# zhouxian/FluidLab

Measured on AMD Instinct MI355X. Metric: MPM substeps/sec (fwd+bwd), 128^3 grid / 200k particles, higher is better.
Workload: dtype f32; 1 GPU; water block 128^3 grid, 200k particles (BASELINE configs[1] inputs), fwd+bwd, evolving (rolling window); nc_start=34727, nc_end=99101, parallelism=1 env, 1 GPU

## Files before the change

### __graft_entry__.py

```python
import os
import subprocess
import sys

ROOT = os.path.dirname(os.path.abspath(__file__))
CSRC = os.path.join(ROOT, 'fluidlab_amd', 'csrc')
HIP_LIB = os.path.join(CSRC, 'libfluidengine_hip.so')
HIPCC_FLAGS = ['--offload-arch=gfx950', '-O3', '-std=c++17', '-shared', '-fPIC', '-munsafe-fp-atomics', '-fno-slp-vectorize']


def _hipcc():
    for c in ('/opt/rocm/bin/hipcc', 'hipcc'):
        if c == 'hipcc' or os.path.exists(c):
            return c


def _source_hash(sources):
    import hashlib
    h = hashlib.sha256(' '.join(HIPCC_FLAGS).encode())
    for s in sources:
        h.update(os.path.basename(s).encode())
        with open(s, 'rb') as f:
            h.update(f.read())
    return h.hexdigest()


def build(force=False):
    srcs = [os.path.join(CSRC, f) for f in ('fe_engine.hip', 'fe_math.h', 'fe_smoke.h', 'fe_mesh.h', 'fe_param_grad.h', 'fe_summary.h', 'fe_task_loss.h')] + \
           [os.path.join(ROOT, 'include', f) for f in ('fluidengine.h', 'fluidengine_ext.h')]
    stamp, want = HIP_LIB + '.srchash', _source_hash(srcs)
    have = open(stamp).read().strip() if os.path.exists(stamp) else ''
    if force or os.environ.get('FE_FORCE_BUILD') == '1' or not os.path.exists(HIP_LIB) or have != want:
        subprocess.check_call([_hipcc()] + HIPCC_FLAGS + ['-o', HIP_LIB, os.path.join(CSRC, 'fe_engine.hip')])
        with open(stamp, 'w') as f:
            f.write(want + '\n')
        print('build: compiled', os.path.relpath(HIP_LIB, ROOT), 'from sources', want[:16])
    else:
        print('build: up to date', os.path.relpath(HIP_LIB, ROOT), 'sources', want[:16])
    subprocess.check_call(['make', '-s', '-C', os.path.join(ROOT, 'oracle')])
    if ROOT not in sys.path:
        sys.path.insert(0, ROOT)
    import fluidlab_amd
    from fluidlab_amd import _capi
    lib = _capi.load_hip()
    missing = lib.missing_symbols()
    assert not missing, f'libfluidengine_hip.so is missing ABI symbols: {missing}'
    assert lib.has_ext, f'libfluidengine_hip.so is missing extension symbols: {lib.missing_ext_symbols()}'


def smoke():
    if ROOT not in sys.path:
        sys.path.insert(0, ROOT)
    sys.path.insert(0, os.path.join(ROOT, 'tests'))
    import numpy as np
    import scenarios as S
    from fluidlab_amd import _capi
    hip = _capi.load_hip()
    oracle = _capi.EngineLib(os.path.join(ROOT, 'oracle', '_build', 'libfe_oracle_f64.so'))
    sc = S.latte_mini()
    a = S.run_latte(hip, sc, device=0)
    b = S.run_latte(oracle, sc)
    assert (a['final']['used'] == b['final']['used']).all()
    assert S.rel_l2(a['final']['x'], b['final']['x']) <= 1e-5, S.rel_l2(a['final']['x'], b['final']['x'])
    assert S.rel_l2(a['step_loss'], b['step_loss']) <= 1e-4
    assert S.cosine(a['action_grad'], b['action_grad']) >= 0.999999
    assert S.rel_l2(a['action_grad'], b['action_grad']) <= 1e-4
    print('smoke ok: backend', hip.backend, 'loss', float(np.sum(a['step_loss'])),
          'action-grad rel L2 vs oracle', S.rel_l2(a['action_grad'], b['action_grad']))


if __name__ == '__main__':
    build(force='--force' in sys.argv)
    if len(sys.argv) > 1 and sys.argv[1] == 'smoke':
        smoke()
```

### fluidlab_amd/_capi.py

```python
import ctypes as C
import os

import numpy as np

_HERE = os.path.dirname(os.path.abspath(__file__))
HIP_LIB_PATH = os.path.join(_HERE, 'csrc', 'libfluidengine_hip.so')

FE_BOUNDARY_CUBE, FE_BOUNDARY_CYLINDER = 0, 1
FE_EFF_PLAIN, FE_EFF_INJECTOR, FE_EFF_AIRCON = 0, 1, 2


class FeEngineError(RuntimeError):
    pass


def _structs(real):
    class FeBoundary(C.Structure):
        _fields_ = [('type', C.c_int), ('lower', real * 3), ('upper', real * 3),
                    ('xz_center', real * 2), ('xz_radius', real), ('restitution', real),
                    ('lock_dims', C.c_int)]

    class FeConfig(C.Structure):
        _fields_ = [('struct_size', C.c_int), ('n_grid', C.c_int), ('n_particles', C.c_int),
                    ('max_substeps_local', C.c_int), ('n_substeps', C.c_int),
# ... 153 lines not shown
    global _hip_lib
    if _hip_lib is None:
        if not os.path.exists(HIP_LIB_PATH):
            raise FeEngineError(
                f'{HIP_LIB_PATH} is missing: build it with `python -c "import __graft_entry__ as g; g.build()"` '
                '(hipcc --offload-arch=gfx950).  There is no CPU fallback.')
        _hip_lib = EngineLib(HIP_LIB_PATH)
    return _hip_lib


class Engine:

    def __init__(self, elib, *, n_grid, n_particles, max_substeps_local, n_substeps,
                 max_action_steps, dt, p_vol, gravity, boundary, device=0):
        self.elib = elib
        self.lib = elib.lib
        self.dtype = elib.dtype
        cfg = elib.FeConfig()
        cfg.struct_size = C.sizeof(elib.FeConfig)
        cfg.n_grid = int(n_grid)
        cfg.n_particles = int(n_particles)
        cfg.max_substeps_local = int(max_substeps_local)
        cfg.n_substeps = int(n_substeps)
        cfg.max_action_steps = int(max_action_steps)
        cfg.dt = float(dt)
        cfg.p_vol = float(p_vol)
        cfg.gravity[:] = [float(g) for g in gravity]
        cfg.boundary = boundary
        cfg.device = int(device)
        self.device = int(device)
        self.cfg = cfg
        self.N = int(n_particles)
        self.n_obs = 0
        self.n_summary_groups = 0
        self.n_task_terms = 0
        self.h = self.lib.fe_create(C.byref(cfg))
        if not self.h:
            raise FeEngineError('fe_create failed: ' + self.lib.fe_last_error(None).decode())
        self.h = C.c_void_p(self.h)

    def close(self):
        if getattr(self, 'h', None):
            self.lib.fe_destroy(self.h)
            self.h = None

    def __del__(self):
        try:
            self.close()
        except Exception:
            pass

    def _ck(self, rc):
        if rc != 0:
            raise FeEngineError(self.lib.fe_last_error(self.h).decode())

    def _r(self, a, shape=None):
        if a is None:
            return None, None
        a = np.ascontiguousarray(a, dtype=self.dtype)
        if shape is not None:
            assert a.shape == tuple(shape), f'expected shape {shape}, got {a.shape}'
        return a, a.ctypes.data_as(C.c_void_p)

    def _i(self, a, shape=None):
        if a is None:
            return None, None
        a = np.ascontiguousarray(a, dtype=np.int32)
        if shape is not None:
            assert a.shape == tuple(shape), f'expected shape {shape}, got {a.shape}'
        return a, a.ctypes.data_as(C.c_void_p)

    def _out(self, a, shape, dtype=None):
        dtype = dtype or self.dtype
        assert isinstance(a, np.ndarray) and a.dtype == dtype and a.flags['C_CONTIGUOUS'] and a.shape == tuple(shape)
        return a.ctypes.data_as(C.c_void_p)

    def sync(self):
        self._ck(self.lib.fe_sync(self.h))

    def set_option(self, name, value):
        self._ck(self.lib.fe_set_option(self.h, name.encode(), float(value)))

    OPTION_NAMES = ('sort_interval', 'item_max', 'grid_store', 'p2g_grad_waves', 'g2p_grad_v', 'loose_max', 'xcd_map', 'write_through',
                    'wave_sort', 'lane_split', 'fold_reorder', 'compact_F', 'fuse_g2p', 'fuse_bwd', 'quad_min_units', 'pgg_quad_min_units', 'quad_max', 'quad_fit', 'pack_units', 'wgrid_cap', 'wgrid_cap_g2p', 'wgrid_cap_pgg', 'ggrid_cap', 'collide_type')

    def get_option(self, name):
        v = C.c_double(0.0)
        self._ck(self.lib.fe_get_option(self.h, name.encode(), C.byref(v)))
        return v.value

    def get_options(self):
        return {n: self.get_option(n) for n in self.OPTION_NAMES}

    def init_particles(self, x, used, mat, mat_cls, mu, lam, rho, body_id):
        N = self.N
        k0, x_ = self._r(x, (N, 3)); k1, u_ = self._i(used, (N,)); k2, m_ = self._i(mat, (N,))
        k3, c_ = self._i(mat_cls, (N,)); k4, mu_ = self._r(mu, (N,)); k5, la_ = self._r(lam, (N,))
        k6, rh_ = self._r(rho, (N,)); k7, b_ = self._i(body_id, (N,))
        self._ck(self.lib.fe_init_particles(self.h, x_, u_, m_, c_, mu_, la_, rh_, b_))

    def substep(self, f, f_global, act):
        self._ck(self.lib.fe_substep(self.h, int(f), int(f_global), int(bool(act))))

    def substep_grad(self, f, f_global, act):
        self._ck(self.lib.fe_substep_grad(self.h, int(f), int(f_global), int(bool(act))))

    def step(self, f0, f_global0, n, act):
        self._ck(self.lib.fe_step(self.h, int(f0), int(f_global0), int(n), int(bool(act))))

    def step_grad(self, f0, f_global0, n, act):
        self._ck(self.lib.fe_step_grad(self.h, int(f0), int(f_global0), int(n), int(bool(act))))

    def get_frame(self, f, x=None, v=None, C_=None, F=None, used=None):
        N = self.N
        px = self._out(x, (N, 3)) if x is not None else None
        pv = self._out(v, (N, 3)) if v is not None else None
        pC = self._out(C_, (N, 3, 3)) if C_ is not None else None
        pF = self._out(F, (N, 3, 3)) if F is not None else None
        pu = self._out(used, (N,), np.int32) if used is not None else None
        self._ck(self.lib.fe_get_frame(self.h, int(f), px, pv, pC, pF, pu))

    def set_frame(self, f, x=None, v=None, C_=None, F=None, used=None):
        N = self.N
        k0, px = self._r(x, (N, 3)); k1, pv = self._r(v, (N, 3)); k2, pC = self._r(C_, (N, 3, 3))
        k3, pF = self._r(F, (N, 3, 3)); k4, pu = self._i(used, (N,))
        self._ck(self.lib.fe_set_frame(self.h, int(f), px, pv, pC, pF, pu))

    @staticmethod
    def _handles(engines):
        arr = (C.c_void_p * len(engines))(*[e.h for e in engines])
        return arr

    @staticmethod
    def step_batch(engines, f0, f_global0, n, act):
        e0 = engines[0]
        e0._ck(e0.lib.fe_step_batch(Engine._handles(engines), len(engines), int(f0), int(f_global0), int(n), int(bool(act))))

    @staticmethod
    def step_grad_batch(engines, f0, f_global0, n, act):
        e0 = engines[0]
        e0._ck(e0.lib.fe_step_grad_batch(Engine._handles(engines), len(engines), int(f0), int(f_global0), int(n), int(bool(act))))

    def copy_frame(self, src, dst):
        self._ck(self.lib.fe_copy_frame(self.h, int(src), int(dst)))

    def copy_grad(self, src, dst):
        self._ck(self.lib.fe_copy_grad(self.h, int(src), int(dst)))

    def reset_grad(self):
        self._ck(self.lib.fe_reset_grad(self.h))

    def reset_grad_till_frame(self, f):
        self._ck(self.lib.fe_reset_grad_till_frame(self.h, int(f)))

    def get_grad(self, f):
        N = self.N
        gx = np.zeros((N, 3), self.dtype); gv = np.zeros((N, 3), self.dtype)
        gC = np.zeros((N, 3, 3), self.dtype); gF = np.zeros((N, 3, 3), self.dtype)
        self._ck(self.lib.fe_get_grad(self.h, int(f), gx.ctypes.data_as(C.c_void_p), gv.ctypes.data_as(C.c_void_p),
                                      gC.ctypes.data_as(C.c_void_p), gF.ctypes.data_as(C.c_void_p)))
        return gx, gv, gC, gF

    @staticmethod
    def _tptr(t):
        return None if t is None else C.c_void_p(t.data_ptr())

    def _torch_fence(self, *tensors):
# ... 243 lines not shown
        d.softness = float(softness)
        self._ck(self.lib.fe_eff_set_mesh(self.h, int(e), C.byref(d), pv))

    def eff_set_act_range(self, e, act_range):
        k, p = self._i(act_range)
        self._ck(self.lib.fe_eff_set_act_range(self.h, int(e), p, int(k.shape[0])))

    def eff_get_state(self, e, f):
        s = np.zeros((8,), self.dtype)
        self._ck(self.lib.fe_eff_get_state(self.h, int(e), int(f), s.ctypes.data_as(C.c_void_p)))
        return s

    def eff_set_state(self, e, f, state8):
        k, p = self._r(state8, (8,))
        self._ck(self.lib.fe_eff_set_state(self.h, int(e), int(f), p))

    def eff_get_vw(self, e, f):
        v = np.zeros((3,), self.dtype); w = np.zeros((3,), self.dtype)
        self._ck(self.lib.fe_eff_get_vw(self.h, int(e), int(f), v.ctypes.data_as(C.c_void_p), w.ctypes.data_as(C.c_void_p)))
        return v, w

    def eff_set_vw(self, e, f, v, w):
        k0, pv = self._r(v, (3,)); k1, pw = self._r(w, (3,))
        self._ck(self.lib.fe_eff_set_vw(self.h, int(e), int(f), pv, pw))

    def eff_set_action(self, e, s, s_global, n_substeps, action):
        k, p = self._r(action)
        self._ck(self.lib.fe_eff_set_action(self.h, int(e), int(s), int(s_global), int(n_substeps), p))

    def eff_set_action_grad(self, e, s, s_global, n_substeps):
        self._ck(self.lib.fe_eff_set_action_grad(self.h, int(e), int(s), int(s_global), int(n_substeps)))

    def eff_apply_action_p(self, e, action_p):
        k, p = self._r(action_p)
        self._ck(self.lib.fe_eff_apply_action_p(self.h, int(e), p))

    def eff_apply_action_p_grad(self, e):
        self._ck(self.lib.fe_eff_apply_action_p_grad(self.h, int(e)))

    def eff_get_action_grad(self, e, s, n, action_dim):
        g = np.zeros((n + 1, action_dim), self.dtype)
        self._ck(self.lib.fe_eff_get_action_grad(self.h, int(e), int(s), int(n), g.ctypes.data_as(C.c_void_p)))
        return g

    def agent_copy_frame(self, src, dst):
        self._ck(self.lib.fe_agent_copy_frame(self.h, int(src), int(dst)))

    def agent_copy_grad(self, src, dst):
        self._ck(self.lib.fe_agent_copy_grad(self.h, int(src), int(dst)))

    def agent_reset_grad_till_frame(self, f):
        self._ck(self.lib.fe_agent_reset_grad_till_frame(self.h, int(f)))

    def agent_set_collector(self, boundary=None, mat=-1):
        self._ck(self.lib.fe_agent_set_collector(self.h, C.byref(boundary) if boundary is not None else None, int(mat)))

    def loss_alloc(self, max_loss_steps):
        self._ck(self.lib.fe_loss_alloc(self.h, int(max_loss_steps)))

    def loss_set_target(self, s, x):
        k, p = self._r(x, (self.N, 3))
        self._ck(self.lib.fe_loss_set_target(self.h, int(s), p))

    def loss_clear(self):
        self._ck(self.lib.fe_loss_clear(self.h))

    def loss_step(self, s, f, matching_mat, weight):
        self._ck(self.lib.fe_loss_step(self.h, int(s), int(f), int(matching_mat), self.elib.real(weight)))

    def loss_step_grad(self, s, f, matching_mat, weight, step_loss_grad):
        self._ck(self.lib.fe_loss_step_grad(self.h, int(s), int(f), int(matching_mat), self.elib.real(weight),
                                            self.elib.real(step_loss_grad)))

    def loss_get(self, n):
        a = np.zeros((n,), self.dtype)
        self._ck(self.lib.fe_loss_get(self.h, a.ctypes.data_as(C.c_void_p), int(n)))
        return a

    def get_stats(self, f):
        st = FeStats()
        self._ck(self.lib.fe_get_stats(self.h, int(f), C.byref(st)))
        return {k: getattr(st, k) for k, _ in FeStats._fields_}

    def get_work_stats(self, f):
        out = (C.c_longlong * 24)()
        if hasattr(self.lib, 'fe_get_work_stats_n'):
            self._ck(self.lib.fe_get_work_stats_n(self.h, int(f), out, 24))
        else:
            self._ck(self.lib.fe_get_work_stats(self.h, int(f), out))
        keys = ('n_items', 'tail_start', 'n_active_blocks', 'n_multi_item_workgroups', 'n_single_item_blocks')
        d = {k: int(out[i]) for i, k in enumerate(keys)}
        d['items_by_size'] = {k: int(out[5 + i]) for i, k in enumerate(('1', '2-4', '5-8', '9-16', '17-32', '33-64', '65-128'))}
        d['n_occupied_blocks'] = int(out[12])
        d['n_loose_particles'] = int(out[13])
        d['n_quad_items'] = int(out[14])
        d['n_quad_units'] = int(out[15])
        d['n_scatter_units'], d['n_gather_units'] = int(out[16]), int(out[17])
        d['packed'] = bool(out[18])
        d['n_leftover_items'] = int(out[19]) + int(out[20])
        d['n_split9_waves'], d['n_split3_waves'] = int(out[21]), int(out[22])
        return d

    def timer_start(self):
        self._ck(self.lib.fe_timer_start(self.h))

    def timer_stop_ms(self):
        ms = self.lib.fe_timer_stop_ms(self.h)
        if ms < 0:
            raise FeEngineError(self.lib.fe_last_error(self.h).decode())
        return ms

    def profile_enable(self, on):
        self._ck(self.lib.fe_profile_enable(self.h, int(bool(on))))

    def profile_read(self, cap=32):
        buf = C.create_string_buffer(4096)
        ms = (C.c_double * cap)()
        cnt = (C.c_longlong * cap)()
        n = self.lib.fe_profile_read(self.h, buf, 4096, ms, cnt, cap)
        names = buf.value.decode().split('\n') if n > 0 else []
        return {names[i]: (ms[i], cnt[i]) for i in range(min(n, len(names)))}
```

### fluidlab_amd/csrc/fe_engine.hip

```cpp
#include <hip/hip_runtime.h>

#include <algorithm>
#include <cstdio>
#include <cstdlib>
#include <cstring>
#include <string>
#include <vector>

#include "../../include/fluidengine.h"
#include "../../include/fluidengine_ext.h"
#include "fe_math.h"

static_assert(sizeof(fe_real) == 4, "the HIP engine is fp32 (macros.py:207-211)");

#define FR_WORDS 25
#define GR_WORDS 24

template <typename T>
struct Plane {
    char* base; unsigned off;
    __host__ __device__ __forceinline__ T& operator[](int s) const { return *(T*)(base + (size_t)(off + (unsigned)s * (unsigned)sizeof(T))); }
    __host__ __device__ __forceinline__ T* ptr() const { return (T*)(base + (size_t)off); }
};
typedef unsigned int u32x4 __attribute__((ext_vector_type(4)));
typedef unsigned int u32x3 __attribute__((ext_vector_type(3)));
__device__ __forceinline__ __amdgpu_buffer_rsrc_t wt_rsrc(void* base) { return __builtin_amdgcn_make_buffer_rsrc(base, 0, -1, 0x00020000); }
__device__ __forceinline__ void wt_store16(void* base, unsigned byte_off, float4 v) {
    const u32x4 u = {__float_as_uint(v.x), __float_as_uint(v.y), __float_as_uint(v.z), __float_as_uint(v.w)};
    __builtin_amdgcn_raw_buffer_store_b128(u, wt_rsrc(base), (int)byte_off, 0, 16);
}
__device__ __forceinline__ void wt_store4(void* base, unsigned byte_off, unsigned v) { __builtin_amdgcn_raw_buffer_store_b32(v, wt_rsrc(base), (int)byte_off, 0, 16); }
struct FrameV {
    Plane<float4> A0, A1, A2; Plane<float> a3, a4, a5; Plane<float4> B0, B1; Plane<float> b2; Plane<int> used;
    int wt;
    int iso;
};
__device__ __forceinline__ void pstore(const FrameV& fr, const Plane<float4>& p, int s, float4 v) {
    if (fr.wt) wt_store16(p.base, p.off + (unsigned)s * 16u, v); else p[s] = v;
}
__device__ __forceinline__ void pstore(const FrameV& fr, const Plane<float>& p, int s, float v) {
    if (fr.wt) wt_store4(p.base, p.off + (unsigned)s * 4u, __float_as_uint(v)); else p[s] = v;
}
__device__ __forceinline__ void pstore(const FrameV& fr, const Plane<int>& p, int s, int v) {
    if (fr.wt) wt_store4(p.base, p.off + (unsigned)s * 4u, (unsigned)v); else p[s] = v;
}
__host__ __device__ inline FrameV frame_view(float* base_, size_t Np_, int wt = 0, int iso = 0) {
    FrameV v;
    v.wt = wt; v.iso = iso;
    char* base = (char*)base_;
    const unsigned Np = (unsigned)Np_;
    v.A0 = {base, 0u}; v.A1 = {base, 16u * Np}; v.A2 = {base, 32u * Np};
    v.a3 = {base, 48u * Np}; v.a4 = {base, 52u * Np}; v.a5 = {base, 56u * Np};
    v.B0 = {base, 60u * Np}; v.B1 = {base, 76u * Np}; v.b2 = {base, 92u * Np};
    v.used = {base, 96u * Np};
    return v;
}

struct PState { float x[3], v[3]; m3 C, F; };
__device__ __forceinline__ void copy_xvC(PState& d, const PState& s) {
#pragma unroll
    for (int a = 0; a < 3; a++) {
        d.x[a] = s.x[a]; d.v[a] = s.v[a];
#pragma unroll
        for (int b = 0; b < 3; b++) d.C.a[a][b] = s.C.a[a][b];
    }
}

__device__ __forceinline__ void load_xvC(const FrameV& fr, int s, PState& p) {
    float4 a0 = fr.A0[s], a1 = fr.A1[s], a2 = fr.A2[s];
    p.x[0] = a0.x; p.x[1] = a0.y; p.x[2] = a0.z; p.v[0] = a0.w; p.v[1] = a1.x; p.v[2] = a1.y;
    p.C.a[0][0] = a1.z; p.C.a[0][1] = a1.w; p.C.a[0][2] = a2.x; p.C.a[1][0] = a2.y; p.C.a[1][1] = a2.z; p.C.a[1][2] = a2.w;
    p.C.a[2][0] = fr.a3[s]; p.C.a[2][1] = fr.a4[s]; p.C.a[2][2] = fr.a5[s];
}
__device__ __forceinline__ void load_F(const FrameV& fr, int s, m3& F) {
    if (fr.iso) {
        const float c = fr.b2[s];
        const float d = fr.iso == 1 ? c : 0.f;
        F.a[0][0] = d; F.a[0][1] = 0.f; F.a[0][2] = 0.f; F.a[1][0] = 0.f; F.a[1][1] = d; F.a[1][2] = 0.f; F.a[2][0] = 0.f; F.a[2][1] = 0.f; F.a[2][2] = c;
        return;
    }
    float4 b0 = fr.B0[s], b1 = fr.B1[s];
    F.a[0][0] = b0.x; F.a[0][1] = b0.y; F.a[0][2] = b0.z; F.a[1][0] = b0.w;
    F.a[1][1] = b1.x; F.a[1][2] = b1.y; F.a[2][0] = b1.z; F.a[2][1] = b1.w; F.a[2][2] = fr.b2[s];
}
__device__ __forceinline__ void store_xvC(const FrameV& fr, int s, const float x[3], const float v[3], const m3& C) {
    const float4 a0 = make_float4(x[0], x[1], x[2], v[0]), a1 = make_float4(v[1], v[2], C.a[0][0], C.a[0][1]), a2 = make_float4(C.a[0][2], C.a[1][0], C.a[1][1], C.a[1][2]);
    if (fr.wt) {
        const unsigned o16 = (unsigned)s * 16u, o4 = (unsigned)s * 4u;
        wt_store16(fr.A0.base, fr.A0.off + o16, a0); wt_store16(fr.A0.base, fr.A1.off + o16, a1); wt_store16(fr.A0.base, fr.A2.off + o16, a2);
        wt_store4(fr.A0.base, fr.a3.off + o4, __float_as_uint(C.a[2][0])); wt_store4(fr.A0.base, fr.a4.off + o4, __float_as_uint(C.a[2][1]));
        wt_store4(fr.A0.base, fr.a5.off + o4, __float_as_uint(C.a[2][2]));
    } else {
        fr.A0[s] = a0; fr.A1[s] = a1; fr.A2[s] = a2;
        fr.a3[s] = C.a[2][0]; fr.a4[s] = C.a[2][1]; fr.a5[s] = C.a[2][2];
// ... 1011 lines not shown
            if (s < S.N) {
                P2GRaw raw;
                bool have = false;
                if (FUSED && prev.used[s]) {
                    const float4 a0 = prev.A0[s];
                    const float xp[3] = {a0.x, a0.y, a0.z};
                    Stencil stp;
                    stencil_make(xp, S.inv_dx, stp);
                    if (stencil_inside(stp, S.n)) {
                        g2p_gather<false, true, true>(S, 0, stp, FU.g_out, 0, raw.p.v, raw.p.C);
#pragma unroll
                        for (int a = 0; a < 3; a++) raw.p.x[a] = xp[a] + S.dt * raw.p.v[a];
                        store_xvC(curw, s, raw.p.x, raw.p.v, raw.p.C);
                        have = true;
                    }
                }
                if (cur.used[s]) {
                    if (WRITE && !FUSED && act && agent.collector && collector_takes(S, cur, nxt, s, T.info, agent)) continue;
                    P2GPrep q;
                    if (FUSED && have) { load_F(cur, s, raw.p.F); raw.info = load_info(S, T.info, s); p2g_compute<WRITE, GENERAL>(S, nxt, s, raw, G, q); }
                    else p2g_prepare<WRITE, GENERAL>(S, cur, nxt, s, T.info, G, q);
                    int none = 0;
                    if (q.inside) p2g_scatter_global<FG>(S, q, G, GS, T.blk_slot, -1, none);
                } else if (WRITE) unused_particle_fwd(S, cur, nxt, s, T.pid_of_slot[s], pool_idx, agent, inj, f);
            }
        }
    }
}
struct P2GArgs { SimP S; float* fr_cur; float* fr_next; TableP T; const int* pool_idx; GridW G; AgentP agent; InjectP inj; int act; int f; GridStore GS; int fiso; FuseP FU; };
template <bool WRITE, bool GENERAL>
__global__ FE_KALIGN __launch_bounds__(WG, GENERAL ? 3 : 4) void k_p2g(SimP S, float* fr_cur, float* fr_next, TableP T, const int* pool_idx, GridW G, AgentP agent, InjectP inj, int act, int f, GridStore GS, int fiso) { p2g_body<WRITE, GENERAL>(S, fr_cur, fr_next, T, pool_idx, G, agent, inj, act, f, GS, fiso); }
template <bool GENERAL>
__global__ FE_KALIGN __launch_bounds__(WG, GENERAL ? 3 : 4) void k_g2p_p2g(SimP S, float* fr_cur, float* fr_next, TableP T, const int* pool_idx, GridW G, AgentP agent, InjectP inj, int act, int f, GridStore GS, int fiso, FuseP FU) { p2g_body<true, GENERAL, true>(S, fr_cur, fr_next, T, pool_idx, G, agent, inj, act, f, GS, fiso, FU); }
template <typename ARGS>
__device__ __forceinline__ const ARGS* fg_args_again() {
    const ARGS* p = (const ARGS*)__builtin_amdgcn_kernarg_segment_ptr();
    asm volatile("" : "+s"(p));
    return p;
}
template <bool GENERAL>
__global__ FE_KALIGN __launch_bounds__(WG, GENERAL ? 3 : 4) void k_p2g_fg(P2GArgs A) {
    p2g_body<true, GENERAL, false, true>(A.S, A.fr_cur, A.fr_next, A.T, A.pool_idx, A.G, A.agent, A.inj, A.act, A.f, A.GS, A.fiso);
    const P2GArgs* B = fg_args_again<P2GArgs>();
    TL(B->S, 3);
    fg_owner_phase<false>(B->S, B->T, B->GS, FgArgs{B->G.fg, B->G.slab, B->G.g_in, B->G.g_out, B->G.blk_list, B->G.blk_count, B->G.blk_flag, B->f});
}
template <bool GENERAL>
__global__ FE_KALIGN __launch_bounds__(WG, GENERAL ? 3 : 4) void k_g2p_p2g_fg(P2GArgs A) {
    p2g_body<true, GENERAL, true, true>(A.S, A.fr_cur, A.fr_next, A.T, A.pool_idx, A.G, A.agent, A.inj, A.act, A.f, A.GS, A.fiso, A.FU);
    const P2GArgs* B = fg_args_again<P2GArgs>();
    TL(B->S, 3);
    fg_owner_phase<false>(B->S, B->T, B->GS, FgArgs{B->G.fg, B->G.slab, B->G.g_in, B->G.g_out, B->G.blk_list, B->G.blk_count, B->G.blk_flag, B->f});
}
template <bool GENERAL>
__global__ FE_KALIGN __launch_bounds__(WG, GENERAL ? 3 : 4) void k_g2p_p2g_b(Batch<P2GArgs> B) { const P2GArgs& A = B.a[blockIdx.y]; p2g_body<true, GENERAL, true>(A.S, A.fr_cur, A.fr_next, A.T, A.pool_idx, A.G, A.agent, A.inj, A.act, A.f, A.GS, A.fiso, A.FU); }
template <bool WRITE, bool GENERAL>
__global__ FE_KALIGN __launch_bounds__(WG, GENERAL ? 3 : 4) void k_p2g_b(Batch<P2GArgs> B) { const P2GArgs& A = B.a[blockIdx.y]; p2g_body<WRITE, GENERAL>(A.S, A.fr_cur, A.fr_next, A.T, A.pool_idx, A.G, A.agent, A.inj, A.act, A.f, A.GS, A.fiso); }


template <bool NODE>
__device__ __forceinline__ bool agent_collide_particle(const SimP& S, const AgentP& agent, int f, const float x[3], float nv[3]) {
    const float sdt = NODE ? 0.f : S.dt;
    bool any = false;
    for (int ei = 0; ei < agent.n; ei++) {
        const EffP& e = agent.e[ei];
        if (!e.has_mesh) continue;
        const float pos[3] = {x[0] + sdt * nv[0], x[1] + sdt * nv[1], x[2] + sdt * nv[2]};
        if (!(pos[1] > agent.collide_min_y)) continue;
        float out[3];
        any |= t_dynamic_collide<float>(e.mesh, e.pos + f * 3, e.quat + f * 4, e.pos + (f + 1) * 3, e.quat + (f + 1) * 4, pos, nv, S.dt, out);
        nv[0] = out[0]; nv[1] = out[1]; nv[2] = out[2];
    }
    return any;
}
#define FE_MAX_STATICS 4
struct NodeWork { int c, ni, nj, nk; float4 gi; float go[3]; float pad; };
struct StaticsP { int n; const SdfP* s; };

template <bool STATICS, bool DYN = false>
__device__ __forceinline__ void node_velocity(const SimP& S, const StaticsP& ST, const float4 gi, int i, int j, int k, float vo[3], float kmul[3],
                                              float (*trace)[3] = nullptr, const AgentP* agent = nullptr, int f = 0, float* vdyn = nullptr,
                                              bool* dyn_hit = nullptr) {
    float inv = 1.f / gi.w;
    vo[0] = inv * gi.x + S.dt * S.g[0];
    vo[1] = inv * gi.y + S.dt * S.g[1];
    vo[2] = inv * gi.z + S.dt * S.g[2];
    float xn[3] = {(float)i * S.dx, (float)j * S.dx, (float)k * S.dx};
    if (STATICS) {
#pragma unroll
        for (int si = 0; si < FE_MAX_STATICS; si++) {
            if (si < ST.n) {
                if (trace) { trace[si][0] = vo[0]; trace[si][1] = vo[1]; trace[si][2] = vo[2]; }
                static_collide(ST.s[si], xn, vo, nullptr);
            }
        }
    }
    if (DYN) {
        if (vdyn) { vdyn[0] = vo[0]; vdyn[1] = vo[1]; vdyn[2] = vo[2]; }
        const bool hit = agent_collide_particle<true>(S, *agent, f, xn, vo);
        if (dyn_hit) *dyn_hit = hit;
    }
    boundary_v(S.bnd, xn, vo, kmul);
}
__device__ __forceinline__ void node_statics_grad(const SimP& S, const StaticsP& ST, int i, int j, int k, const float (*trace)[3], float g[3]) {
    float xn[3] = {(float)i * S.dx, (float)j * S.dx, (float)k * S.dx};
#pragma unroll
    for (int si = FE_MAX_STATICS - 1; si >= 0; si--) {
        if (si < ST.n) {
            float vin[3] = {trace[si][0], trace[si][1], trace[si][2]};
            static_collide(ST.s[si], xn, vin, g);
        }
    }
}

__device__ __forceinline__ int2 nbr_record(const TableP& T, int e, int lane) {
    return lane < 27 ? T.nbr[e * 27 + lane] : make_int2(0, 0);
}
template <int NPL>
__device__ __forceinline__ float4 gather_slabs(const float4* __restrict__ slab, const int2 mine, int lane) {
    const int o[3] = {lane >> 4, (lane >> 2) & 3, lane & 3};
    int a0[8], n[8];
    float4 v0[8], v1[8];
#pragma unroll
    for (int c = 0; c < 8; c++) {
        int nbr = 0, si = 0;
        bool valid = true;
#pragma unroll
        for (int d = 0; d < 3; d++) {
            const bool other = (c >> d) & 1;
            valid = valid && (!other || o[d] <= 1);
            nbr = nbr * 3 + (other ? 0 : 1);
            si = si * SLAB_T + o[d] + (other ? 4 : 0);
        }
        const int f = __shfl(mine.x, nbr, 64), k = __shfl(mine.y, nbr, 64);
        n[c] = valid ? k : 0;
        a0[c] = valid ? (NPL == 4 ? f * SLAB_N + si : f * (SLAB_N * 16) + si * 12) : 0;
    }
    const __amdgpu_buffer_rsrc_t rs = wt_rsrc((void*)slab);
    auto ld = [&](int at) -> float4 {
        if (NPL == 4) return slab[at];
        const u32x3 u = __builtin_amdgcn_raw_buffer_load_b96(rs, at, 0, 0);
        return make_float4(__uint_as_float(u.x), __uint_as_float(u.y), __uint_as_float(u.z), 0.f);
    };
    constexpr int STRIDE = NPL == 4 ? SLAB_N : SLAB_N * 16;
#pragma unroll
    for (int c = 0; c < 8; c++) {
        const bool h0 = n[c] > 0, h1 = n[c] > 2;
        const float4 a = ld(h0 ? a0[c] : 0);
        const float4 b = ld(h1 ? a0[c] + 2 * STRIDE : 0);
        v0[c] = make_float4(h0 ? a.x : 0.f, h0 ? a.y : 0.f, h0 ? a.z : 0.f, h0 ? a.w : 0.f);
        v1[c] = make_float4(h1 ? b.x : 0.f, h1 ? b.y : 0.f, h1 ? b.z : 0.f, h1 ? b.w : 0.f);
    }
    float4 acc = make_float4(0.f, 0.f, 0.f, 0.f);
#pragma unroll
    for (int c = 0; c < 8; c++) {
        acc.x += v0[c].x; acc.y += v0[c].y; acc.z += v0[c].z; acc.w += v0[c].w;
        acc.x += v1[c].x; acc.y += v1[c].y; acc.z += v1[c].z; acc.w += v1[c].w;
        for (int k = 4; k < n[c]; k += 2) {
            const float4 v = ld(a0[c] + k * STRIDE);
            acc.x += v.x; acc.y += v.y; acc.z += v.z; acc.w += v.w;
        }
    }
    return acc;
}

__device__ __forceinline__ int static_entry(int wave) {
    const int G = gridDim.x;
    if ((G & 127) != 0) return blockIdx.x * 4 + wave;
    const int j = blockIdx.x >> 3;
// ... 1699 lines not shown
            const int n = wave_iscan((l >= 0 && l < SORT_HB) ? hist[l] : 0);
            if (lane == 63 && n > 0) atomicAdd(&bcnt[(base >> 6) + j], n);
        }
    }
    if (tid == 255 && hist[SORT_HB] > 0) atomicAdd(&bcnt[S.ncell >> 6], hist[SORT_HB]);
    __syncthreads();
    {
        const int k0 = kmin;
        int c[SORT_HB / 256], b[SORT_HB / 256];
#pragma unroll
        for (int i = 0; i < SORT_HB / 256; i++) c[i] = hist[tid + 256 * i];
        const int ct = tid == 0 ? hist[SORT_HB] : 0;
        int bt = 0;
#pragma unroll
        for (int i = 0; i < SORT_HB / 256; i++) { b[i] = 0; if (c[i] > 0) b[i] = atomicAdd(&cnt[k0 + tid + 256 * i], c[i]); }
        if (ct > 0) bt = atomicAdd(&cnt[S.ncell], ct);
#pragma unroll
        for (int i = 0; i < SORT_HB / 256; i++) if (c[i] > 0) hist[tid + 256 * i] = b[i];
        if (ct > 0) hist[SORT_HB] = bt;
    }
    __syncthreads();
    if (local) r += hist[rel];
    if (valid) { key[s] = kk; rank[s] = r; }
}

struct BlkWork { int k, full, single, left, last; };
__device__ __forceinline__ BlkWork block_work(int n, int ITEM_MAX) {
    BlkWork w;
    w.k = (n + ITEM_MAX - 1) / ITEM_MAX;
    w.full = w.k > 1 ? w.k >> 1 : 0;
    w.single = w.k == 1 ? 1 : 0;
    w.left = (w.k > 1 && (w.k & 1)) ? 1 : 0;
    w.last = n - (w.k - 1) * ITEM_MAX;
    return w;
}

#define SORT_BLK_WG 1024
#define NSUM 11
#define PART_STRIDE 16
struct BlkSums { int v[NSUM]; };
__device__ __forceinline__ void blk_accumulate(BlkSums& a, int n, int ITEM_MAX, int loose_max, int quad_max) {
    const bool occ = n > 0, loose = occ && n <= loose_max, dense = occ && !loose;
    const BlkWork w = block_work(n > 0 ? n : 1, ITEM_MAX);
    const bool small = w.last <= quad_max;
    a.v[5] += occ ? 1 : 0;
    a.v[1] += loose ? n : 0;
    a.v[0] += dense ? n : 0;
    a.v[2] += dense ? w.k : 0;
    a.v[3] += dense ? w.full : 0;
    a.v[4] += (dense && w.single && !small) ? 1 : 0;
    a.v[6] += (dense && w.single && small && w.last > FE_SPLIT3_MAX) ? 1 : 0;
    a.v[9] += (dense && w.single && small && w.last <= FE_SPLIT3_MAX && w.last > FE_SPLIT9_MAX) ? 1 : 0;
    a.v[10] += (dense && w.single && small && w.last <= FE_SPLIT9_MAX) ? 1 : 0;
    a.v[7] += (dense && w.left && !small) ? 1 : 0;
    a.v[8] += (dense && w.left && small) ? 1 : 0;
}
__device__ __forceinline__ int4 blk_ask4(const int* __restrict__ bcnt) { return *(const int4*)(bcnt + blockIdx.x * SORT_BLK_WG + threadIdx.x * 4); }
__device__ __forceinline__ BlkSums blk_sums4(const int4 n4, int nblk, int ITEM_MAX, int loose_max, int quad_max, int n[4]) {
    const int b0 = blockIdx.x * SORT_BLK_WG + threadIdx.x * 4;
    n[0] = b0 < nblk ? n4.x : 0; n[1] = b0 + 1 < nblk ? n4.y : 0; n[2] = b0 + 2 < nblk ? n4.z : 0; n[3] = b0 + 3 < nblk ? n4.w : 0;
    BlkSums m = {{0, 0, 0, 0, 0, 0, 0, 0, 0, 0, 0}};
#pragma unroll
    for (int u = 0; u < 4; u++) blk_accumulate(m, n[u], ITEM_MAX, loose_max, quad_max);
    return m;
}
__device__ __forceinline__ void wg_scan6(const BlkSums& m, int (*sh)[NSUM], int ex[NSUM], int tot[NSUM]) {
    const int lane = threadIdx.x & 63, wave = __builtin_amdgcn_readfirstlane(threadIdx.x >> 6);
#pragma unroll
    for (int k = 0; k < NSUM; k++) {
        const int incl = wave_iscan(m.v[k]);
        ex[k] = incl - m.v[k];
        if (lane == 63) sh[wave][k] = incl;
    }
    __syncthreads();
#pragma unroll
    for (int k = 0; k < NSUM; k++) {
        int before = 0, all = 0;
#pragma unroll
        for (int w = 0; w < 4; w++) { const int t = sh[w][k]; all += t; if (w < wave) before += t; }
        ex[k] += before; tot[k] = all;
    }
    __syncthreads();
}
template <bool ONE>
__device__ __forceinline__ bool sort_side_jobs(int nblk, int nb, const int* __restrict__ bcnt, int blk_wgs, int scan_wgs, int* cnt, int* start, int* nact, int* active, int* blk_slot,
                                               int* act_done, int act_target, int* meta) {
    const int lane = threadIdx.x & 63;
    if ((int)blockIdx.x >= blk_wgs + scan_wgs) {
        const int b = (blockIdx.x - blk_wgs - scan_wgs) * 256 + threadIdx.x;
        bool on = false;
        {
            const bool inb = b < nblk;
            const int bb = inb ? b : 0;
            const int bi = bb / (nb * nb), bj = (bb / nb) % nb, bk = bb % nb;
            int v[27];
            unsigned okm = 0;
#pragma unroll
            for (int t = 0; t < 27; t++) {
                const int i2 = bi + t / 9 - 1, j2 = bj + (t / 3) % 3 - 1, k2 = bk + t % 3 - 1;
                const bool ok = (unsigned)i2 < (unsigned)nb && (unsigned)j2 < (unsigned)nb && (unsigned)k2 < (unsigned)nb;
                okm |= (ok ? 1u : 0u) << t;
                v[t] = bcnt[ok ? (i2 * nb + j2) * nb + k2 : bb];
            }
            int any = 0;
#pragma unroll
            for (int t = 0; t < 27; t++) any |= ((okm >> t) & 1u) ? v[t] : 0;
            on = inb && any > 0;
        }
        const unsigned long long wm = __ballot(on);
        if (wm) {
            int base = 0;
            if (lane == 0) base = atomicAdd(nact, __popcll(wm));
            base = __shfl(base, 0, 64);
            if (on) { const int e = base + __popcll(wm & ((1ull << lane) - 1ull)); active[e] = b; blk_slot[b] = e; }
        }
        if (!on && b < nblk) blk_slot[b] = -1;
        if (ONE) {
            __syncthreads();
            if (threadIdx.x == 0 && __hip_atomic_fetch_add(act_done, 1, __ATOMIC_RELAXED, __HIP_MEMORY_SCOPE_AGENT) == act_target - 1)
                meta[2] = __hip_atomic_load(nact, __ATOMIC_RELAXED, __HIP_MEMORY_SCOPE_AGENT);
        }
        return true;
    }
    if ((int)blockIdx.x >= blk_wgs) {
        const int g = (blockIdx.x - blk_wgs) * 4 + (threadIdx.x >> 6);
        const int bl = g * 16 + (lane & 15);
        const unsigned occ = (unsigned)__ballot(lane < 16 && bl < nblk && bcnt[bl] > 0);
        if (!occ) return true;
        int4 c[4];
#pragma unroll
        for (int i = 0; i < 4; i++) {
            const int b = g * 16 + i * 4 + (lane >> 4);
            c[i] = make_int4(0, 0, 0, 0);
            if (((occ >> (4 * i)) & 15u) && b < nblk) c[i] = *(const int4*)(cnt + (size_t)b * 64 + (lane & 15) * 4);
        }
#pragma unroll
        for (int i = 0; i < 4; i++) {
            if (!((occ >> (4 * i)) & 15u)) continue;
            const int b = g * 16 + i * 4 + (lane >> 4);
            const int s0 = c[i].x, s1 = s0 + c[i].y, s2 = s1 + c[i].z, s3 = s2 + c[i].w;
            const int ex = row_iscan(s3) - s3;
            if (b < nblk && ((occ >> (4 * i + (lane >> 4))) & 1u)) {
                *(int4*)(start + (size_t)b * 64 + (lane & 15) * 4) = make_int4(ex, ex + s0, ex + s1, ex + s2);
                if (s3) *(int4*)(cnt + (size_t)b * 64 + (lane & 15) * 4) = make_int4(0, 0, 0, 0);
            }
        }
        return true;
    }
    return false;
}
__global__ __launch_bounds__(256) void k_sort_blk_partial(int nblk, int nb, int ITEM_MAX, int loose_max, int quad_max, const int* __restrict__ bcnt, int* partial,
                                                          int blk_wgs, int scan_wgs, int* cnt, int* start, int* nact, int* active, int* blk_slot) {
    __shared__ int sh[4][NSUM];
    if (sort_side_jobs<false>(nblk, nb, bcnt, blk_wgs, scan_wgs, cnt, start, nact, active, blk_slot, nullptr, 0, nullptr)) return;
    int n[4], ex[NSUM], tot[NSUM];
    const BlkSums m = blk_sums4(blk_ask4(bcnt), nblk, ITEM_MAX, loose_max, quad_max, n);
    wg_scan6(m, sh, ex, tot);
#pragma unroll
    for (int k = 0; k < NSUM; k++) if ((int)threadIdx.x == k) partial[blockIdx.x * PART_STRIDE + k] = tot[k];
}
__device__ __forceinline__ void sort_blk_final_body(int (*sh)[NSUM], const int4 n4, const BlkSums& pb, const BlkSums& pa, int nblk, int nb, int ncell, int ITEM_MAX, int loose_max, int quad_max,
                                                    int* cnt, int* start, int4* items, int2* pairs, int* singles, int* singles_c, int2* blk_first, int* blk_base, const int* __restrict__ nact, int* meta) {
    const int tid = threadIdx.x;
    int n[4], ex[NSUM], tot[NSUM];
    const BlkSums m = blk_sums4(n4, nblk, ITEM_MAX, loose_max, quad_max, n);
    int exb[NSUM], before[NSUM], exa[NSUM], total[NSUM];
    wg_scan6(pb, sh, exb, before);
    wg_scan6(pa, sh, exa, total);
    wg_scan6(m, sh, ex, tot);
    if (blockIdx.x == 0 && tid == 0) { meta[0] = total[2]; meta[1] = total[0]; if (nact) meta[2] = *nact; meta[3] = total[3]; meta[4] = total[4]; meta[6] = total[5]; meta[7] = total[0] + total[1]; meta[8] = total[6] + total[9] + total[10];
                                       meta[11] = total[7]; meta[12] = total[8]; }
    const int b0 = blockIdx.x * SORT_BLK_WG + tid * 4;
    if (b0 > nblk) return;
    int D = before[0] + ex[0], L = total[0] + before[1] + ex[1], bi = before[2] + ex[2], bm = before[3] + ex[3];
    int p_tb = before[4] + ex[4], p_lb = total[4] + before[7] + ex[7], p_ls = total[4] + total[7] + before[8] + ex[8];
    const int ts0 = total[4] + total[7] + total[8];
    int p_ts = ts0 + before[6] + ex[6], p_t3 = ts0 + total[6] + before[9] + ex[9], p_t9 = ts0 + total[6] + total[9] + before[10] + ex[10];
    int p_bo = ts0 + before[6] + ex[6] + before[9] + ex[9] + before[10] + ex[10];
    int2 bf[4];
    int base[4] = {0, 0, 0, 0};
#pragma unroll
    for (int u = 0; u < 4; u++) {
        const int b = b0 + u, nn = n[u];
        bf[u] = make_int2(0, 0);
        if (b > nblk) continue;
        if (b == nblk) { base[u] = total[0] + total[1]; start[ncell] = 0; cnt[ncell] = 0; continue; }
        if (nn <= 0) continue;
        if (nn <= loose_max) { base[u] = L; L += nn; continue; }
        const BlkWork w = block_work(nn, ITEM_MAX);
        bf[u] = make_int2(bi, w.k);
        base[u] = D;
        const bool small = w.last <= quad_max;
        if (w.single) {
            if (!small) { singles[p_tb] = bi; singles_c[p_tb++] = bi; }
            else {
                singles[p_bo++] = bi;
                if (w.last > FE_SPLIT3_MAX) singles_c[p_ts++] = bi;
                else if (w.last > FE_SPLIT9_MAX) singles_c[p_t3++] = bi;
                else singles_c[p_t9++] = bi;
            }
        }
        if (w.left) { if (small) { singles[p_ls] = bi + w.k - 1; singles_c[p_ls++] = bi + w.k - 1; } else { singles[p_lb] = bi + w.k - 1; singles_c[p_lb++] = bi + w.k - 1; } }
        for (int j = 0; j < w.full; j++) pairs[bm++] = make_int2(bi + 2 * j, bi + 2 * j + 1);
        const int pk = BLK_PACK(b / (nb * nb), (b / nb) % nb, b % nb);
        for (int o = 0; o < nn; o += ITEM_MAX) items[bi++] = make_int4(pk, D + o, min(ITEM_MAX, nn - o), 0);
        D += nn;
    }
    *(int4*)(blk_base + b0) = make_int4(base[0], base[1], base[2], base[3]);
    if (b0 + 3 < nblk) { *(int4*)(blk_first + b0) = make_int4(bf[0].x, bf[0].y, bf[1].x, bf[1].y); *(int4*)(blk_first + b0 + 2) = make_int4(bf[2].x, bf[2].y, bf[3].x, bf[3].y); }
    else for (int u = 0; u < 4; u++) if (b0 + u < nblk) blk_first[b0 + u] = bf[u];
}
__global__ __launch_bounds__(256) void k_sort_blk_final(int nblk, int nb, int ncell, int ITEM_MAX, int loose_max, int quad_max, const int* __restrict__ bcnt, int* cnt, int* start,
                                                        const int* __restrict__ partial, int4* items, int2* pairs, int* singles, int* singles_c, int2* blk_first, int* blk_base, const int* __restrict__ nact, int* meta) {
    __shared__ int sh[4][NSUM];
    const int tid = threadIdx.x;
    const int4 n4 = blk_ask4(bcnt);
    BlkSums pb = {{0, 0, 0, 0, 0, 0, 0, 0, 0, 0, 0}}, pa = {{0, 0, 0, 0, 0, 0, 0, 0, 0, 0, 0}};
    for (int w = tid; w < (int)gridDim.x; w += 256) {
#pragma unroll
        for (int k = 0; k < NSUM; k++) { const int t = partial[w * PART_STRIDE + k]; pa.v[k] += t; if (w < (int)blockIdx.x) pb.v[k] += t; }
    }
    sort_blk_final_body(sh, n4, pb, pa, nblk, nb, ncell, ITEM_MAX, loose_max, quad_max, cnt, start, items, pairs, singles, singles_c, blk_first, blk_base, nact, meta);
}
struct SortScanSync { int* ready; int ready_target; int* act_done; int act_target; };
__global__ __launch_bounds__(256) void k_sort_blk_scan(int nblk, int nb, int ncell, int ITEM_MAX, int loose_max, int quad_max, const int* __restrict__ bcnt, int* partial, int blk_wgs, int scan_wgs,
                                                       int* cnt, int* start, int* nact, int* active, int* blk_slot, int4* items, int2* pairs, int* singles, int* singles_c, int2* blk_first,
                                                       int* blk_base, int* meta, SortScanSync Y) {
    __shared__ int sh[4][NSUM];
    if (sort_side_jobs<true>(nblk, nb, bcnt, blk_wgs, scan_wgs, cnt, start, nact, active, blk_slot, Y.act_done, Y.act_target, meta)) return;
    const int tid = threadIdx.x;
    const int4 n4 = blk_ask4(bcnt);
    {
        int n[4], ex[NSUM], tot[NSUM];
        const BlkSums m = blk_sums4(n4, nblk, ITEM_MAX, loose_max, quad_max, n);
        wg_scan6(m, sh, ex, tot);
#pragma unroll
        for (int k = 0; k < NSUM; k++) if (tid == k) __hip_atomic_store(partial + blockIdx.x * PART_STRIDE + k, tot[k], __ATOMIC_RELAXED, __HIP_MEMORY_SCOPE_AGENT);
    }
    asm volatile("s_waitcnt vmcnt(0)" ::: "memory");
    __syncthreads();
    if (tid == 0) {
        __hip_atomic_fetch_add(Y.ready, 1, __ATOMIC_RELAXED, __HIP_MEMORY_SCOPE_AGENT);
        while ((int)(__hip_atomic_load(Y.ready, __ATOMIC_RELAXED, __HIP_MEMORY_SCOPE_AGENT) - Y.ready_target) < 0) __builtin_amdgcn_s_sleep(1);
    }
    __syncthreads();
    BlkSums pb = {{0, 0, 0, 0, 0, 0, 0, 0, 0, 0, 0}}, pa = {{0, 0, 0, 0, 0, 0, 0, 0, 0, 0, 0}};
    for (int w = tid; w < blk_wgs; w += 256) {
#pragma unroll
        for (int k = 0; k < NSUM; k++) { const int t = __hip_atomic_load(partial + w * PART_STRIDE + k, __ATOMIC_RELAXED, __HIP_MEMORY_SCOPE_AGENT); pa.v[k] += t; if (w < (int)blockIdx.x) pb.v[k] += t; }
    }
    sort_blk_final_body(sh, n4, pb, pa, nblk, nb, ncell, ITEM_MAX, loose_max, quad_max, cnt, start, items, pairs, singles, singles_c, blk_first, blk_base, nullptr, meta);
}

struct UnitLists { int nF, tB, lB, lS, tS; };
__device__ __forceinline__ int unit_count(const UnitLists& u, bool pack, int x, int n_tail) {
    const int nsing = u.tB + u.lB + u.lS + u.tS;
    return u.nF + (pack ? (nsing - x + 1) >> 1 : u.lB + u.lS + ((u.tB + u.tS - x + 1) >> 1)) + ((x + 3) >> 2) + n_tail;
}
__device__ __forceinline__ void build_unit_list(int gtid, int nth, int N, int xcd_on, const int4* __restrict__ items, const int2* __restrict__ pairs,
                                                const int* __restrict__ singles, int tail_start, const UnitLists L, bool pack, int x, int* n_slots_out, int* n_work_out, UnitRec* units, int units_cap) {
    const int nsing = L.tB + L.lB + L.lS + L.tS, n_left = L.lB + L.lS;
    const int n_alone = pack ? 0 : n_left;
    const int n_two = pack ? nsing - x : L.tB + L.tS - x;
    const int n_pairs = L.nF + n_alone + ((n_two + 1) >> 1), n_quads = (x + 3) >> 2, n_tail = (N - tail_start + WG - 1) / WG;
    const int n_work = n_pairs + n_quads + n_tail;
    const int per_xcd = xcd_on >= 2 ? (((n_work + xcd_on - 1) / xcd_on + 7) >> 3) * xcd_on : (n_work + 7) >> 3;
    const int n_slots = per_xcd * 8 < units_cap ? per_xcd * 8 : units_cap;
    if (gtid == 0) { *n_slots_out = n_slots; *n_work_out = n_work; }
    auto two = [&](int j) { return singles[pack ? j : (j < L.tB ? j : j + n_left)]; };
    for (int w = gtid; w < n_slots; w += nth) {
        const int u = xcd_item(w, per_xcd, xcd_on);
        UnitRec un;
        un.a = make_int4(0, 0, -2, 0); un.b = un.c = un.d = make_int4(0, 0, 0, -1);
        if (u < n_pairs) {
            int ia, ib, same;
            if (u < L.nF) { const int2 pr = pairs[u]; ia = pr.x; ib = pr.y; same = 1; }
            else if (u < L.nF + n_alone) { ia = singles[L.tB + (u - L.nF)]; ib = -1; same = 1; }
            else { const int q = 2 * (u - L.nF - n_alone); ia = two(q); ib = q + 1 < n_two ? two(q + 1) : -1; same = 0; }
            un.a = items[ia]; un.a.w = ia | (same << 30);
            if (ib >= 0) { un.b = items[ib]; un.b.w = ib; }
        } else if (u < n_pairs + n_quads) {
            const int q = nsing - x + 4 * (u - n_pairs), nq = min(4, nsing - q);
            { const int ii = singles[q]; un.a = items[ii]; un.a.w = ii | QUAD_BIT; }
            if (nq > 1) { const int ii = singles[q + 1]; un.b = items[ii]; un.b.w = ii; }
            if (nq > 2) { const int ii = singles[q + 2]; un.c = items[ii]; un.c.w = ii; }
            if (nq > 3) { const int ii = singles[q + 3]; un.d = items[ii]; un.d.w = ii; }
        } else if (u < n_work) un.a = make_int4(0, tail_start + (u - n_pairs - n_quads) * WG, -1, 0);
        units[w] = un;
    }
}
__device__ __forceinline__ void build_units_dev(int gtid, int nth, int nb, int N, int xcd_on, int quad_min_units, int quad_fit, int pack_units, int pgg_quad_min_units, const int4* __restrict__ items, const int2* __restrict__ pairs,
                                                const int* __restrict__ singles, const int* __restrict__ singles_c, const int2* __restrict__ blk_first, const int* __restrict__ active,
                                                int* meta, UnitRec* units, UnitRec* units_p, int units_cap, int2* nbr, int* expected) {
    const int tail_start = meta[1], n_active = meta[2];
    const UnitLists L = {meta[3], meta[4], meta[11], meta[12], meta[8]};
    const int n_tail = (N - tail_start + WG - 1) / WG;
    const int U0 = unit_count(L, false, 0, n_tail);
    bool pack = false; int x = 0;
    if (U0 > quad_fit && quad_fit > 0) {
        const int U1 = unit_count(L, true, 0, n_tail), small = L.lS + L.tS;
        const int need = U1 > quad_fit ? 4 * (U1 - quad_fit) + 4 : 0;
        if (pack_units > 0 && need <= small) { pack = true; x = need; }
        else if (U0 > quad_min_units) { pack = pack_units > 1; x = pack ? small : L.tS; }
        else pack = pack_units > 1;
    } else if (U0 > quad_min_units) x = L.tS;
    if (gtid == 0) { meta[10] = (x + 3) >> 2; meta[13] = pack ? 1 : 0; }
    if (gtid == 0) meta[16] = (x > 0 && U0 > pgg_quad_min_units) ? 1 : 0;
    build_unit_list(gtid, nth, N, xcd_on, items, pairs, singles_c, tail_start, L, pack, x, meta + 5, meta + 14, units, units_cap);
    build_unit_list(gtid, nth, N, xcd_on, items, pairs, singles, tail_start, L, false, 0, meta + 9, meta + 15, units_p, units_cap);
    for (int t0 = gtid; t0 < n_active * 27; t0 += 4 * nth) {
        int b[4];
#pragma unroll
        for (int u = 0; u < 4; u++) { const int t = t0 + u * nth; b[u] = t < n_active * 27 ? active[t / 27] : 0; }
        int2 v[4];
#pragma unroll
        for (int u = 0; u < 4; u++) {
            const int t = t0 + u * nth, n = t % 27;
            const int i2 = b[u] / (nb * nb) + n / 9 - 1, j2 = (b[u] / nb) % nb + (n / 3) % 3 - 1, k2 = b[u] % nb + n % 3 - 1;
            v[u] = make_int2(0, 0);
            if (t < n_active * 27 && (unsigned)i2 < (unsigned)nb && (unsigned)j2 < (unsigned)nb && (unsigned)k2 < (unsigned)nb) v[u] = blk_first[(i2 * nb + j2) * nb + k2];
        }
#pragma unroll
        for (int u = 0; u < 4; u++) { const int t = t0 + u * nth; if (t < n_active * 27) nbr[t] = v[u]; }
    }
    if (expected) for (int e = gtid; e < n_active; e += nth) {
        const int b = active[e], bi = b / (nb * nb), bj = (b / nb) % nb, bk = b % nb;
        int cnt[27];
#pragma unroll
        for (int n = 0; n < 27; n++) {
            const int i2 = bi + n / 9 - 1, j2 = bj + (n / 3) % 3 - 1, k2 = bk + n % 3 - 1;
            const bool ok = (unsigned)i2 < (unsigned)nb && (unsigned)j2 < (unsigned)nb && (unsigned)k2 < (unsigned)nb;
            cnt[n] = ok ? blk_first[(i2 * nb + j2) * nb + k2].y : 0;
        }
        int sum = 0;
// ... 388 lines not shown
}
__global__ __launch_bounds__(256) void k_stats_count(int ncells, unsigned char* node_mark, unsigned long long* counters) {
    const int lane = threadIdx.x & 63;
    const int b = (blockIdx.x * blockDim.x + threadIdx.x) >> 6;
    if (b * 64 >= ncells) return;
    bool t = node_mark[b * 64 + lane] != 0;
    node_mark[b * 64 + lane] = 0;
    unsigned long long m = __ballot(t);
    if (lane == 0 && m) { atomicAdd(&counters[1], (unsigned long long)__popcll(m)); atomicAdd(&counters[2], 1ull); }
}

#include "fe_param_grad.h"
#include "fe_summary.h"
#include "fe_task_loss.h"

enum { KID_P2G = 0, KID_GRID, KID_G2P, KID_P2G_RE, KID_GRID_KEEP, KID_G2P_GRAD, KID_GRID_GRAD, KID_P2G_GRAD, KID_SORT, KID_REORDER_GRAD, KID_SORT_COUNT, KID_SORT_SCAN, KID_SORT_ACTIVE, KID_SORT_PERM, KID_G2P_P2G, KID_PGG_G2PG, KID_PARAM_GRAD, KID_COUNT };
static const char* KNAMES[KID_COUNT] = {"p2g", "grid_op", "g2p", "p2g_recompute", "grid_op_keep", "g2p_grad", "grid_op_grad", "p2g_grad", "sort", "reorder_grad", "sort_count", "sort_scan", "sort_active", "sort_perm", "g2p_p2g", "pgg_g2pg", "param_grad"};

struct EffHost {
    EffP p;
    std::vector<int> act_id;
    std::vector<int> act_range;
};

struct FeEngine {
    FeConfig cfg;
    int N = 0, Np = 0, L = 0, n = 0, nb = 0;
    int device = 0;
    hipStream_t stream = nullptr;
    SimP S;
    float* frames = nullptr; size_t frame_stride = 0;
    std::vector<float*> frame_ptr;
    float* grads = nullptr;
    float* grad_ptr[3] = {nullptr, nullptr, nullptr};
    struct Table { int* pid = nullptr; float4* info = nullptr; int2* pairs = nullptr; int* singles = nullptr; int4* items = nullptr; int* meta = nullptr; int2* blk_first = nullptr; int* active = nullptr; int* blk_slot = nullptr; int* slot_of_pid = nullptr; UnitRec* units = nullptr; UnitRec* units_p = nullptr; int2* nbr = nullptr; unsigned long long* arrive = nullptr;  bool has_expected = false;  };
    int loose_max = 0;
    std::vector<int> gs_host; bool gs_host_valid = false;
    float4* gstore = nullptr; int* gs_flag = nullptr; int gs_cap = 0;
    unsigned char *ent_touched = nullptr, *ent_dirty = nullptr; unsigned stamp = 0;
    unsigned char *gs_live = nullptr, *cur_live = nullptr;
    float4* slab = nullptr;
    std::vector<Table> tables;
    std::vector<int> tbl_of_frame;
    int gtbl[2] = {-1, -1};
    std::vector<char> fiso;
    bool gcompact[2] = {false, false};
    bool gpartial[2] = {false, false};
    int n_cus = 256;
    bool compact_F = true;
    int fuse_bwd = 1;
    bool fuse_g2p = true;
    int fuse_grid = 0;
    FgDev fg_host = {nullptr, nullptr, nullptr, nullptr, nullptr}; FgDev* fg_dev = nullptr;
    unsigned fg_started = 0;
    bool tail_used = true;
    int tbl_bank = 0, last_sorted_f = -1;
    int sort_keys_in_g2p = 1;
    int keys_frame = -1;
    bool sort_scratch_dirty = false;
    int p2g_grad_waves = 4;
    int pack_units = 2;
    int quad_fit = 1024;
    int quad_min_units = 1400;
    int pgg_quad_min_units = 1800;
    int quad = QUAD_MAX;
    int g2p_grad_v = 3;
    int item_max = ITEM_MAX_CAP;
    int sort_interval = 10;
    size_t items_cap = 0, units_cap = 0;
    int *sort_key = nullptr, *sort_rank = nullptr, *sort_cnt = nullptr, *sort_start = nullptr, *sort_pid = nullptr, *sort_bcnt = nullptr, *sort_partial = nullptr, *sort_base = nullptr, *sort_nact = nullptr;
    int sort_one_scan = 0, scan_ready = 0, scan_act = 0;
    int* slow_dev = nullptr;
    int* frame_slow_dev = nullptr;
    float4* pinfo = nullptr; int* pool_idx = nullptr;
    std::vector<int> mat_host;
    float *g_in = nullptr, *gg_out = nullptr;
    float4 *g_out = nullptr, *gg_in = nullptr;
    bool all_simple_liquid = false;
    std::vector<SdfP> statics_host; std::vector<float*> statics_vox; SdfP* statics_dev = nullptr;
    struct SmokeState* smoke = nullptr;
    unsigned char* hit_dev = nullptr;
    int* hit_list = nullptr; int* hit_count = nullptr;
    NodeWork* node_work = nullptr; int* node_work_count = nullptr;
    int ggrid_cap = 1024;
    bool fold_reorder = true;
    int wgrid_cap_pgg = 2048;
    int wgrid_cap_g2p = 2048;
    int wgrid_cap = 2048;
    int collide_type = 1;
    BoundaryP* collector_dev = nullptr; bool has_collector = false; int collector_mat = -1;
    int inject_till = -1; float collide_min_y = -1e30f;
    bool prof_fine = false;
    bool param_grad = false;
    double* pg_acc = nullptr;
    int* obs_pids = nullptr; int obs_n = 0;
    float *obs_x = nullptr, *obs_v = nullptr; int* obs_u = nullptr;
    int* sum_group = nullptr; int sum_n_groups = 0;
    FeSumAcc* sum_partial = nullptr; FeFrameSummary* sum_out = nullptr;
    int tl_steps = 0; double *tl_step_loss = nullptr, *tl_term_loss = nullptr;
    FeLossTerm tl_terms[FE_TASK_LOSS_MAX_TERMS]; int tl_n = 0; FeLossTerm* tl_terms_dev = nullptr;
    bool tl_has_sep = false, tl_has_ref = false; int tl_n_pair = 0;
    float* tl_ref = nullptr; bool tl_ref_set = false;
    double* tl_partial = nullptr; size_t tl_partial_cap = 0;
    int* tl_cnt = nullptr;
    int task_pair_chunk = 0;
    bool has_mesh_effector = false; std::vector<float*> mesh_vox;
    bool has_rigid = false; int n_bodies = 0;
    RigidBody* bodies_dev = nullptr;
    int* body_start = nullptr; int* body_pids = nullptr;
    int *blk_flag = nullptr, *blk_list = nullptr, *blk_count = nullptr, *err_dev = nullptr;
    float* stage_r = nullptr; int* stage_i = nullptr;
    unsigned char* node_mark = nullptr; unsigned long long* counters = nullptr;
    std::vector<EffHost> effs;
    EffP* effs_dev = nullptr;
    int loss_steps = 0; float *tgt = nullptr, *chamfer = nullptr, *step_loss = nullptr;
    size_t bytes = 0;
    std::string err;
    hipEvent_t ev_t0 = nullptr, ev_t1 = nullptr, ev_batch = nullptr;
    hipStream_t own_stream = nullptr;
    bool prof_on = false;
    std::vector<hipEvent_t> prof_ev; std::vector<int> prof_kid; size_t prof_used = 0;
    double prof_ms[KID_COUNT] = {0}; long long prof_n[KID_COUNT] = {0};
#ifdef FE_TIMELINE
    unsigned long long* tl_dev = nullptr;
#endif

    float* frame(int f) { return frame_ptr[f]; }
    float*& spare_frame() { return frame_ptr[L + 1]; }
    float* grad(int f) { return grad_ptr[f & 1]; }
    size_t grad_words() const { return (size_t)GR_WORDS * Np + Np; }
    TableP tableP(int id) const { TableP t; t.pid_of_slot = tables[id].pid; t.info = tables[id].info; t.meta = tables[id].meta; t.active = tables[id].active; t.blk_slot = tables[id].blk_slot; t.units = tables[id].units; t.units_p = tables[id].units_p; t.units_cap = (int)units_cap; t.nbr = tables[id].nbr; t.arrive = tables[id].arrive; return t; }
    int* expected_of(int id) const { return (int*)(tables[id].arrive + (size_t)nb * nb * nb); }
    const int* pid_of(int f) const { return tables[tbl_of_frame[f]].pid; }
};

static std::string g_create_err;

static hipError_t hipMemcpyOnStream(FeEngine* h, void* dst, const void* src, size_t bytes, hipMemcpyKind kind);

#define FAIL(h, msg) do { (h)->err = (msg); return 1; } while (0)
#define FE_ENTRY(h) do { if ((h) != nullptr) (void)hipSetDevice((h)->device); } while (0)
#define HIPCK(h, call) do { hipError_t e_ = (call); if (e_ != hipSuccess) { (h)->err = std::string(#call) + ": " + hipGetErrorString(e_); return 1; } } while (0)
#define CHECK_FRAME(h, f) do { if ((f) < 0 || (f) > (h)->L) FAIL(h, "frame index out of range"); } while (0)
#define CHECK_EFF(h, e) do { if ((e) < 0 || (e) >= (int)(h)->effs.size()) FAIL(h, "effector index out of range"); } while (0)

static hipError_t hipMemcpyOnStream(FeEngine* h, void* dst, const void* src, size_t bytes, hipMemcpyKind kind) {
    hipError_t e = hipMemcpyAsync(dst, src, bytes, kind, h->stream);
    if (e != hipSuccess) return e;
    return hipStreamSynchronize(h->stream);
}

namespace {

template <typename T>
int dev_alloc(FeEngine* h, T** p, size_t count, bool zero = true) {
    size_t bytes = count * sizeof(T);
    if (bytes == 0) bytes = sizeof(T);
    HIPCK(h, hipMalloc((void**)p, bytes));
    if (zero) HIPCK(h, hipMemsetAsync(*p, 0, bytes, h->stream));
    h->bytes += bytes;
    return 0;
}

BoundaryP to_boundary(const FeBoundary& b) {
    BoundaryP r;
    r.type = b.type;
    for (int i = 0; i < 3; i++) { r.lower[i] = b.lower[i]; r.upper[i] = b.upper[i]; }
    r.cx = b.xz_center[0]; r.cz = b.xz_center[1]; r.radius = b.xz_radius; r.restitution = b.restitution; r.lock_dims = b.lock_dims;
    return r;
}

AgentP agent_params(FeEngine* h) {
    AgentP a; a.n = (int)h->effs.size(); a.inj = 0; a.e = h->effs_dev; a.collide_min_y = h->collide_min_y;
    a.collector = h->has_collector ? h->collector_dev : nullptr; a.collector_mat = h->collector_mat;
    a.hit = h->hit_dev;
    for (size_t i = 0; i < h->effs.size(); i++) if (h->effs[i].p.type == FE_EFF_INJECTOR) a.inj = (int)i;
    return a;
}

inline dim3 pgrid(FeEngine* h) { return dim3((h->N + 255) / 256); }
inline dim3 wgrid(FeEngine* h) { int g = (h->N + 63) / 64 + 8; if (g < 512) g = 512; return dim3(g < h->wgrid_cap ? g : h->wgrid_cap); }
inline dim3 wgrid_g2p(FeEngine* h) { int g = (h->N + 63) / 64 + 8; if (g < 512) g = 512; return dim3(g < h->wgrid_cap_g2p ? g : h->wgrid_cap_g2p); }
inline dim3 wgrid_pgg(FeEngine* h) { int g = (h->N + 63) / 64 + 8; if (g < 512) g = 512; return dim3(g < h->wgrid_cap_pgg ? g : h->wgrid_cap_pgg); }
inline dim3 ggrid(FeEngine* h) { int blocks = h->nb * h->nb * h->nb; int g = (blocks + 3) / 4; return dim3(g < h->ggrid_cap ? g : h->ggrid_cap); }

void prof_drain(FeEngine* h);
void prof_begin(FeEngine* h, int kid) {
#ifdef FE_TIMELINE
    if (!h->tl_dev) { (void)hipMalloc((void**)&h->tl_dev, sizeof(unsigned long long) * KID_COUNT * TL_WGS * 9); }
    h->S.tl = h->tl_dev + (size_t)kid * TL_WGS * 9;
    (void)hipMemsetAsync(h->S.tl, 0, sizeof(unsigned long long) * TL_WGS * 9, h->stream);
#endif
    if (!h->prof_on) return;
    if (h->prof_used >= 8192) prof_drain(h);
    if (h->prof_used + 2 > h->prof_ev.size()) {
        for (int i = 0; i < 256; i++) { hipEvent_t e; (void)hipEventCreate(&e); h->prof_ev.push_back(e); }
    }
    h->prof_kid.push_back(kid);
    (void)hipEventRecord(h->prof_ev[h->prof_used++], h->stream);
}
void prof_end(FeEngine* h) {
    if (!h->prof_on) return;
    (void)hipEventRecord(h->prof_ev[h->prof_used++], h->stream);
}
void prof_drain(FeEngine* h) {
    if (h->prof_used == 0) return;
    (void)hipStreamSynchronize(h->stream);
    for (size_t i = 0; i + 1 < h->prof_used; i += 2) {
        float ms = 0;
        (void)hipEventElapsedTime(&ms, h->prof_ev[i], h->prof_ev[i + 1]);
        int kid = h->prof_kid[i / 2];
        h->prof_ms[kid] += ms; h->prof_n[kid]++;
    }
    h->prof_used = 0; h->prof_kid.clear();
}

int find_injector(FeEngine* h) {
    for (size_t i = 0; i < h->effs.size(); i++) if (h->effs[i].p.type == FE_EFF_INJECTOR) return (int)i;
    return -1;
}

int make_inject(FeEngine* h, int f, int f_global, int act, bool forward, InjectP& inj) {
    inj.on = 0; inj.act_id = 0; inj.row = 0; inj.flux = 0;
    int ie = find_injector(h);
    if (ie < 0) return 0;
    EffHost& E = h->effs[ie];
    if (!act || (h->inject_till >= 0 && f_global >= h->inject_till)) {
        if (forward) E.act_id[f + 1] = E.act_id[f];
        return 0;
    }
    if (E.act_range.empty()) FAIL(h, "injector has no act_range");
    int row = E.p.locally_random ? f : f_global;
    if (row < 0 || row >= E.p.random_length) FAIL(h, "injector random_vector row out of range");
    if (forward) {
        if (E.act_id[f] + E.p.flux > (int)E.act_range.size()) FAIL(h, "too many particles added");
        E.act_id[f + 1] = E.act_id[f] + E.p.flux;
    }
    inj.on = 1; inj.act_id = E.act_id[f]; inj.row = row; inj.flux = E.p.flux;
    return 0;
}

int check_async(FeEngine* h);

void build_units(FeEngine* h, FeEngine::Table& t) {
    hipLaunchKernelGGL(k_build_units, dim3(256), dim3(256), 0, h->stream, h->nb, h->N, h->S.xcd, t.items, t.pairs, t.singles, t.blk_first, t.active, t.meta,
                       t.units, t.units_p, (int)h->units_cap, t.nbr, (h->fuse_grid & 3) ? (int*)(t.arrive + (size_t)h->nb * h->nb * h->nb) : (int*)nullptr);
    t.has_expected = (h->fuse_grid & 3) != 0;
}
int ensure_table(FeEngine* h, int id) {
    if ((int)h->tables.size() <= id) h->tables.resize(id + 1);
    FeEngine::Table& t = h->tables[id];
    if (t.pid) return 0;
    const size_t nblk = (size_t)h->nb * h->nb * h->nb;
    if (id == 0) t.info = h->pinfo;
    else if (dev_alloc(h, &t.info, h->Np)) return 1;
    if (dev_alloc(h, &t.pairs, h->items_cap) || dev_alloc(h, &t.singles, 2 * h->items_cap)) return 1;
    if (dev_alloc(h, &t.pid, h->Np) || dev_alloc(h, &t.items, h->items_cap) || dev_alloc(h, &t.meta, 24) ||
        dev_alloc(h, &t.blk_first, nblk) || dev_alloc(h, &t.active, nblk) || dev_alloc(h, &t.blk_slot, nblk) || dev_alloc(h, &t.slot_of_pid, h->Np) ||
        dev_alloc(h, &t.units, h->units_cap, false) || dev_alloc(h, &t.units_p, h->units_cap, false) || dev_alloc(h, &t.nbr, nblk * 27, false) ||
        dev_alloc(h, &t.arrive, nblk + (nblk + 1) / 2)) return 1;
    HIPCK(h, hipMemsetAsync(t.blk_slot, 0xff, sizeof(int) * nblk, h->stream));
    if (id == 0) build_units(h, t);
    return 0;
}

int reorder_grad(FeEngine* h, int slot, int to) {
    const int from = h->gtbl[slot];
    if (from == to || from < 0) { if (from >= 0) h->gtbl[slot] = to; return 0; }
    prof_begin(h, KID_REORDER_GRAD);
    hipLaunchKernelGGL(k_perm_reorder, pgrid(h), dim3(256), 0, h->stream, h->N, (size_t)h->Np, h->grad_ptr[2], h->grad_ptr[slot],
                       h->tables[to].pid, h->tables[from].slot_of_pid);
    std::swap(h->grad_ptr[2], h->grad_ptr[slot]);
    prof_end(h);
    h->gtbl[slot] = to;
    return 0;
}

int grad_table_for_frame(FeEngine* h, int f) {
    if (h->gtbl[f & 1] < 0) h->gtbl[f & 1] = h->tbl_of_frame[f];
    return h->gtbl[f & 1];
}

int use_static_table(FeEngine*, int) { return 0; }

inline int quad_max(FeEngine* h) { return h->quad; }
int sort_frame(FeEngine* h, int f) {
    if (f <= h->last_sorted_f) h->tbl_bank ^= 1;
    h->last_sorted_f = f;
    const int id_new = 1 + f + h->tbl_bank * (h->L + 1), id_old = h->tbl_of_frame[f];
    if (ensure_table(h, id_new)) return 1;
    for (int slot = 0; slot < 2; slot++)
        if (h->gtbl[slot] == id_new && reorder_grad(h, slot, 0)) return 1;
    FeEngine::Table& tn = h->tables[id_new];
    const int ncell = h->S.ncell;
    const bool fine = h->prof_on && h->prof_fine;
    if (!fine) prof_begin(h, KID_SORT);
    const int n_pwg = (int)pgrid(h).x;
    const int nblk = h->nb * h->nb * h->nb;
    if (fine) prof_begin(h, KID_SORT_COUNT);
    const bool have_keys = h->keys_frame == f && h->sort_scratch_dirty;
    if (!have_keys && h->sort_scratch_dirty) {
        HIPCK(h, hipMemsetAsync(h->sort_cnt, 0, sizeof(int) * ((size_t)ncell + 1), h->stream));
        HIPCK(h, hipMemsetAsync(h->sort_bcnt, 0, sizeof(int) * (size_t)(((nblk + 1 + SORT_BLK_WG - 1) / SORT_BLK_WG) * SORT_BLK_WG), h->stream));
    }
    h->keys_frame = -1; h->sort_scratch_dirty = false;
    if (!have_keys)
    hipLaunchKernelGGL(k_sort_count, dim3(n_pwg + SORT_CLR_WGS), dim3(256), 0, h->stream, h->S, h->frame(f), n_pwg, h->sort_key, h->sort_rank, h->sort_cnt, h->sort_bcnt,
                       tn.active, tn.meta, tn.blk_slot, h->sort_nact);
    if (fine) { prof_end(h); prof_begin(h, KID_SORT_SCAN); }
    const int blk_wgs = (nblk + 1 + SORT_BLK_WG - 1) / SORT_BLK_WG, scan_wgs = (nblk + 63) / 64, act_wgs = (nblk + 255) / 256;
    if (h->sort_one_scan && blk_wgs <= 2 * h->n_cus) {
        h->scan_ready += blk_wgs; h->scan_act += act_wgs;
        const SortScanSync Y = {h->sort_nact + 1, h->scan_ready, h->sort_nact + 2, h->scan_act};
        hipLaunchKernelGGL(k_sort_blk_scan, dim3(blk_wgs + scan_wgs + act_wgs), dim3(256), 0, h->stream, nblk, h->nb, ncell, h->item_max, h->loose_max, quad_max(h), h->sort_bcnt, h->sort_partial,
                           blk_wgs, scan_wgs, h->sort_cnt, h->sort_start, h->sort_nact, tn.active, tn.blk_slot, tn.items, tn.pairs, tn.singles, tn.singles + h->items_cap, tn.blk_first,
                           h->sort_base, tn.meta, Y);
    } else {
        hipLaunchKernelGGL(k_sort_blk_partial, dim3(blk_wgs + scan_wgs + act_wgs), dim3(256), 0, h->stream, nblk, h->nb, h->item_max, h->loose_max, quad_max(h), h->sort_bcnt, h->sort_partial,
                           blk_wgs, scan_wgs, h->sort_cnt, h->sort_start, h->sort_nact, tn.active, tn.blk_slot);
        hipLaunchKernelGGL(k_sort_blk_final, dim3(blk_wgs), dim3(256), 0, h->stream, nblk, h->nb, ncell, h->item_max, h->loose_max, quad_max(h), h->sort_bcnt, h->sort_cnt, h->sort_start, h->sort_partial,
                           tn.items, tn.pairs, tn.singles, tn.singles + h->items_cap, tn.blk_first, h->sort_base, h->sort_nact, tn.meta);
    }
    if (fine) { prof_end(h); prof_begin(h, KID_SORT_PERM); }
    int* pid_dst = id_old == id_new ? h->sort_pid : tn.pid;
    const UnitsArgs U = {h->sort_bcnt, h->nb, h->S.xcd, h->quad_min_units, h->quad_fit, h->pack_units, h->pgg_quad_min_units, tn.items, tn.pairs, tn.singles, tn.singles + h->items_cap, tn.blk_first, tn.active, tn.meta, tn.units, tn.units_p, (int)h->units_cap, tn.nbr, (h->fuse_grid & 3) ? (int*)(tn.arrive + (size_t)nblk) : (int*)nullptr};
    tn.has_expected = (h->fuse_grid & 3) != 0;
    hipLaunchKernelGGL(k_sort_apply, dim3(n_pwg + SORT_UNIT_WGS), dim3(256), 0, h->stream, h->N, (size_t)h->Np, n_pwg, h->sort_key, h->sort_rank, h->sort_start, h->sort_base,
                       h->tables[id_old].pid, pid_dst, tn.slot_of_pid, h->pinfo, tn.info, h->spare_frame(), h->frame(f), U, h->S.uni, h->fiso[f] ? 1 : 0);
    if (id_old == id_new) HIPCK(h, hipMemcpyAsync(tn.pid, h->sort_pid, sizeof(int) * h->Np, hipMemcpyDeviceToDevice, h->stream));
    prof_end(h);
    std::swap(h->frame_ptr[f], h->spare_frame());
    h->tbl_of_frame[f] = id_new;
    return 0;
}

StaticsP statics_p(FeEngine* h) { StaticsP p; p.n = (int)h->statics_host.size(); p.s = h->statics_dev; return p; }

GridStore grid_store(FeEngine* h) {
    GridStore g; g.data = h->gstore; g.flag = h->gs_flag; g.cap = h->gs_cap;
    g.touched = h->ent_touched; g.dirty = h->ent_dirty; g.live = h->gs_live; g.cur = h->cur_live; g.stamp = (unsigned char)(1 + h->stamp % 255);
    return g;
}

inline int* bcount(FeEngine* h, int f) { return h->blk_count + (f & 1); }
inline float4* gout(FeEngine* h, int f) { return h->g_out + (size_t)(f & 1) * h->S.ncell; }
inline float4* ggin(FeEngine* h, int f) { return h->gg_in + (size_t)(f & 1) * h->S.ncell; }
GridW grid_w(FeEngine* h, int f) {
    GridW g; g.g_in = h->g_in; g.slab = h->slab; g.ncell = h->S.ncell; g.frame_slow = h->frame_slow_dev; g.blk_flag = h->blk_flag; g.blk_list = h->blk_list; g.blk_count = bcount(h, f); g.err = h->err_dev; g.slow = h->slow_dev;
    g.fg = h->fg_dev; g.g_out = gout(h, f);
    return g;
}

inline bool grid_collide(FeEngine* h) { return h->has_mesh_effector && (h->collide_type & 2); }
inline bool particle_collide(FeEngine* h) { return h->has_mesh_effector && (h->collide_type & 1); }

template <bool KEEP>
void launch_grid(FeEngine* h, const TableP& T, int f, const AgentP& ag) {
#define LAUNCH_GRID(ST_, DY_) hipLaunchKernelGGL(HIP_KERNEL_NAME(k_grid<KEEP, ST_, DY_>), ggrid(h), dim3(256), 0, h->stream, h->S, T, h->slab, h->g_in, gout(h, f), \
                           h->blk_list, bcount(h, f), h->blk_flag, grid_store(h), f, h->frame_slow_dev, statics_p(h), ag)
    if (grid_collide(h)) { if (h->statics_host.empty()) LAUNCH_GRID(false, true); else LAUNCH_GRID(true, true); }
    else { if (h->statics_host.empty()) LAUNCH_GRID(false, false); else LAUNCH_GRID(true, false); }
#undef LAUNCH_GRID
}

inline int fwd_iso(FeEngine* h, int f) { return (h->fiso[f] ? 1 : 0) | ((h->all_simple_liquid && h->compact_F) ? 2 : 0); }

inline bool fusable_fwd(FeEngine* h, int f) {
    return h->fuse_g2p && f > 0 && !(h->sort_interval > 0 && f % h->sort_interval == 0) && !particle_collide(h) && !h->has_rigid && !h->has_collector;
}
inline bool fuse_grid_possible(FeEngine* h, int t) {
    return (h->fuse_grid & 3) != 0 && h->sort_interval > 0 && t > 0 && h->loose_max == 0 && h->statics_host.empty() && !h->has_mesh_effector &&
           h->gs_cap == h->nb * h->nb * h->nb && h->tables[t].has_expected;
}
inline bool fuse_grid_ok(FeEngine* h, int f) { return fuse_grid_possible(h, h->tbl_of_frame[f]) && ((h->fuse_grid & 3) >= 2 || !h->tail_used); }
inline void fg_launch_begin(FeEngine* h) { h->S.fg_base = h->fg_started; h->S.fg_nowait = (h->fuse_grid & 4) ? 1 : 0; }
inline void fg_launch_end(FeEngine* h, dim3 grid) { h->fg_started += grid.x; }
int substep_fwd(FeEngine* h, int f, int f_global, int act, bool g2p_pending = false, bool defer_g2p = false) {
    h->gs_host_valid = false;
    h->stamp++;
    InjectP inj;
    if (make_inject(h, f, f_global, act, true, inj)) return 1;
    if (h->sort_interval > 0 && f % h->sort_interval == 0) { if (sort_frame(h, f)) return 1; h->tail_used = false; }
    h->tbl_of_frame[f + 1] = h->tbl_of_frame[f];
    use_static_table(h, h->tbl_of_frame[f]);
    const TableP T = h->tableP(h->tbl_of_frame[f]);
    AgentP ag = agent_params(h);
    const int fiso = fwd_iso(h, f);
    const bool fg = fuse_grid_ok(h, f);
    if (inj.on) h->tail_used = true;
    if (fg) fg_launch_begin(h);
    if (g2p_pending) {
        const FuseP FU = {h->frame(f - 1), gout(h, f - 1), h->slow_dev, bcount(h, f - 1)};
        prof_begin(h, KID_G2P_P2G);
        if (fg) {
            const P2GArgs A = {h->S, h->frame(f), h->frame(f + 1), T, h->pool_idx, grid_w(h, f), ag, inj, act, f, grid_store(h), h->all_simple_liquid ? fiso : 0, FU};
            if (h->all_simple_liquid) hipLaunchKernelGGL((k_g2p_p2g_fg<false>), wgrid(h), dim3(WG), 0, h->stream, A);
            else hipLaunchKernelGGL((k_g2p_p2g_fg<true>), wgrid(h), dim3(WG), 0, h->stream, A);
        } else if (h->all_simple_liquid)
            hipLaunchKernelGGL((k_g2p_p2g<false>), wgrid(h), dim3(WG), 0, h->stream, h->S, h->frame(f), h->frame(f + 1), T,
                               h->pool_idx, grid_w(h, f), ag, inj, act, f, grid_store(h), fiso, FU);
        else
            hipLaunchKernelGGL((k_g2p_p2g<true>), wgrid(h), dim3(WG), 0, h->stream, h->S, h->frame(f), h->frame(f + 1), T,
                               h->pool_idx, grid_w(h, f), ag, inj, act, f, grid_store(h), 0, FU);
        prof_end(h);
    } else {
    prof_begin(h, KID_P2G);
    if (fg) {
        const P2GArgs A = {h->S, h->frame(f), h->frame(f + 1), T, h->pool_idx, grid_w(h, f), ag, inj, act, f, grid_store(h), h->all_simple_liquid ? fiso : 0, FuseP{nullptr, nullptr, nullptr, nullptr}};
        if (h->all_simple_liquid) hipLaunchKernelGGL((k_p2g_fg<false>), wgrid(h), dim3(WG), 0, h->stream, A);
        else hipLaunchKernelGGL((k_p2g_fg<true>), wgrid(h), dim3(WG), 0, h->stream, A);
    } else if (h->all_simple_liquid)
        hipLaunchKernelGGL((k_p2g<true, false>), wgrid(h), dim3(WG), 0, h->stream, h->S, h->frame(f), h->frame(f + 1), T,
                           h->pool_idx, grid_w(h, f), ag, inj, act, f, grid_store(h), fiso);
    else
        hipLaunchKernelGGL((k_p2g<true, true>), wgrid(h), dim3(WG), 0, h->stream, h->S, h->frame(f), h->frame(f + 1), T,
                           h->pool_idx, grid_w(h, f), ag, inj, act, f, grid_store(h), 0);
    prof_end(h);
    }
    if (fg) fg_launch_end(h, wgrid(h));
    h->fiso[f + 1] = (fiso & 2) != 0;
    if (!fg) {
    prof_begin(h, KID_GRID);
    launch_grid<false>(h, T, f, ag);
    prof_end(h);
    }
    if (defer_g2p) return 0;
    prof_begin(h, KID_G2P);
    const bool sortkey = h->sort_keys_in_g2p && h->sort_interval > 0 && (f + 1) % h->sort_interval == 0 && !h->has_rigid;
    if (sortkey) {
        if (h->sort_scratch_dirty) {
            HIPCK(h, hipMemsetAsync(h->sort_cnt, 0, sizeof(int) * ((size_t)h->S.ncell + 1), h->stream));
            HIPCK(h, hipMemsetAsync(h->sort_bcnt, 0, sizeof(int) * (size_t)((((size_t)h->nb * h->nb * h->nb + 1 + SORT_BLK_WG - 1) / SORT_BLK_WG) * SORT_BLK_WG), h->stream));
        }
        const SortKeyP K = {h->sort_key, h->sort_rank, h->sort_cnt, h->sort_bcnt, h->sort_nact};
        if (particle_collide(h))
            hipLaunchKernelGGL(k_g2p_sortkey<true>, wgrid_g2p(h), dim3(WG), 0, h->stream, h->S, h->frame(f), h->frame(f + 1), T, gout(h, f), bcount(h, f), h->slow_dev, ag, f, K);
        else
            hipLaunchKernelGGL(k_g2p_sortkey<false>, wgrid_g2p(h), dim3(WG), 0, h->stream, h->S, h->frame(f), h->frame(f + 1), T, gout(h, f), bcount(h, f), h->slow_dev, ag, f, K);
        h->keys_frame = f + 1; h->sort_scratch_dirty = true;
    } else if (particle_collide(h))
        hipLaunchKernelGGL(k_g2p<true>, wgrid_g2p(h), dim3(WG), 0, h->stream, h->S, h->frame(f), h->frame(f + 1), T, gout(h, f), bcount(h, f), h->slow_dev, ag, f);
    else
        hipLaunchKernelGGL(k_g2p<false>, wgrid_g2p(h), dim3(WG), 0, h->stream, h->S, h->frame(f), h->frame(f + 1), T, gout(h, f), bcount(h, f), h->slow_dev, ag, f);
    prof_end(h);
    if (h->has_rigid) {
        hipLaunchKernelGGL(k_rigid_body<false>, dim3(h->n_bodies), dim3(256), 0, h->stream, h->S, h->frame(f), h->frame(f + 1), (float*)nullptr,
                           h->tables[h->tbl_of_frame[f]].slot_of_pid, h->body_start, h->body_pids, h->bodies_dev);
    }
    return 0;
}

int fetch_gs_flags(FeEngine* h) {
    if (h->gs_cap > 0 && !h->gs_host_valid) {
        h->gs_host.resize(h->L + 1);
        HIPCK(h, hipMemcpyAsync(h->gs_host.data(), h->gs_flag, sizeof(int) * (h->L + 1), hipMemcpyDeviceToHost, h->stream));
        HIPCK(h, hipStreamSynchronize(h->stream));
        h->gs_host_valid = true;
    }
    return 0;
}
inline bool fusable_bwd(FeEngine* h, int f) {
    if (!h->all_simple_liquid && h->fuse_bwd < 2 && h->Np / 256 > 2 * 3 * (size_t)h->n_cus) return false;
    return h->fuse_bwd && f > 0 && h->g2p_grad_v == 3 && (h->p2g_grad_waves >= 4 || !h->all_simple_liquid) && !particle_collide(h) && !h->has_rigid && !h->has_collector &&
           h->tbl_of_frame[f - 1] == h->tbl_of_frame[f] && h->tbl_of_frame[f] >= 0 && h->gs_cap > 0 && h->gs_host_valid && h->gs_host[f - 1] != 0;
}
int substep_bwd(FeEngine* h, int f, int f_global, int act, int next_f = -1, bool compact_out = false, bool g2p_done = false, bool fuse_next = false) {
    InjectP inj;
    if (make_inject(h, f, f_global, act, false, inj)) return 1;
    const int t = h->tbl_of_frame[f];
    if (!g2p_done && h->gpartial[(f + 1) & 1]) FAIL(h, "the adjoint of frame f + 1 is incomplete: a fused fe_step_grad passed it on in registers (only the adjoint of a call's first frame is defined afterwards; option fuse_bwd = 0 keeps every frame's)");
    if (reorder_grad(h, (f + 1) & 1, t)) return 1;
    use_static_table(h, t);
    const TableP T = h->tableP(t);
    AgentP ag = agent_params(h);
    InjectP noinj = {0, 0, 0, 0};
    if (fetch_gs_flags(h)) return 1;
    const bool stored = h->gs_cap > 0 && h->gs_host[f] != 0;
    if (!g2p_done) {
    if (!stored) {
    h->stamp++;
    prof_begin(h, KID_P2G_RE);
    if (h->all_simple_liquid)
        hipLaunchKernelGGL((k_p2g<false, false>), wgrid(h), dim3(WG), 0, h->stream, h->S, h->frame(f), h->frame(f + 1), T,
                           h->pool_idx, grid_w(h, f), ag, noinj, 0, f, grid_store(h), h->fiso[f] ? 1 : 0);
    else
        hipLaunchKernelGGL((k_p2g<false, true>), wgrid(h), dim3(WG), 0, h->stream, h->S, h->frame(f), h->frame(f + 1), T,
                           h->pool_idx, grid_w(h, f), ag, noinj, 0, f, grid_store(h), 0);
    prof_end(h);
    prof_begin(h, KID_GRID_KEEP);
    launch_grid<true>(h, T, f, ag);
    prof_end(h);
    }
    h->stamp++;
    if (h->has_rigid) {
        hipLaunchKernelGGL(k_rigid_body<true>, dim3(h->n_bodies), dim3(256), 0, h->stream, h->S, h->frame(f), h->frame(f + 1), h->grad(f + 1),
                           h->tables[t].slot_of_pid, h->body_start, h->body_pids, h->bodies_dev);
    }
    prof_begin(h, KID_G2P_GRAD);
    if (particle_collide(h)) {
        HIPCK(h, hipMemsetAsync(h->hit_count, 0, sizeof(int), h->stream));
        hipLaunchKernelGGL(k_collide_list, pgrid(h), dim3(256), 0, h->stream, h->S, h->frame(f), f, ag, h->hit_list, h->hit_count);
        hipLaunchKernelGGL(k_collide_grad, dim3(std::min((h->N + 15) / 16, 2048)), dim3(256), 0, h->stream, h->S, h->frame(f), h->grad(f + 1), gout(h, f), T, grid_store(h), f, ag,
                           h->hit_list, h->hit_count);
    }
    if (h->g2p_grad_v == 2) hipLaunchKernelGGL(k_g2p_grad2<3>, wgrid(h), dim3(WG), 0, h->stream, h->S, h->frame(f), h->grad(f + 1), h->grad(f), T, gout(h, f), h->gg_out, h->slab, h->slow_dev, grid_store(h), f, ag);
    else hipLaunchKernelGGL(k_g2p_grad2<4>, wgrid(h), dim3(WG), 0, h->stream, h->S, h->frame(f), h->grad(f + 1), h->grad(f), T, gout(h, f), h->gg_out, h->slab, h->slow_dev, grid_store(h), f, ag);
    prof_end(h);
    }
    prof_begin(h, KID_GRID_GRAD);
#define LAUNCH_GRID_GRAD(ST_, DY_) hipLaunchKernelGGL(HIP_KERNEL_NAME(k_grid_grad<ST_, DY_>), ggrid(h), dim3(256), 0, h->stream, h->S, T, h->slab, h->g_in, h->gg_out, \
                           ggin(h, f), h->blk_list, bcount(h, f), h->blk_flag, grid_store(h), f, statics_p(h), ag, h->node_work, h->node_work_count)
    if (grid_collide(h)) {
        if (!h->node_work && (dev_alloc(h, &h->node_work, (size_t)h->S.ncell, false) || dev_alloc(h, &h->node_work_count, 1))) return 1;
        HIPCK(h, hipMemsetAsync(h->node_work_count, 0, sizeof(int), h->stream));
        if (h->statics_host.empty()) LAUNCH_GRID_GRAD(false, true); else LAUNCH_GRID_GRAD(true, true);
        const dim3 wg((unsigned)std::min((h->S.ncell + 15) / 16, 1024));
        if (h->statics_host.empty()) hipLaunchKernelGGL(k_grid_collide_grad<false>, wg, dim3(256), 0, h->stream, h->S, ggin(h, f), f, statics_p(h), ag, h->node_work, h->node_work_count);
        else hipLaunchKernelGGL(k_grid_collide_grad<true>, wg, dim3(256), 0, h->stream, h->S, ggin(h, f), f, statics_p(h), ag, h->node_work, h->node_work_count);
    } else { if (h->statics_host.empty()) LAUNCH_GRID_GRAD(false, false); else LAUNCH_GRID_GRAD(true, false); }
    prof_end(h);
    if (h->param_grad) {
        prof_begin(h, KID_PARAM_GRAD);
        if (h->all_simple_liquid) hipLaunchKernelGGL(k_param_grad<false>, pgrid(h), dim3(256), 0, h->stream, h->S, h->frame(f), T, ggin(h, f), h->fiso[f] ? 1 : 0, (float)h->cfg.p_vol, h->pg_acc);
        else hipLaunchKernelGGL(k_param_grad<true>, pgrid(h), dim3(256), 0, h->stream, h->S, h->frame(f), T, ggin(h, f), 0, (float)h->cfg.p_vol, h->pg_acc);
        prof_end(h);
    }
    const int t_next = (h->fold_reorder && next_f >= 0) ? h->tbl_of_frame[next_f] : t;
    const bool fold = t_next != t && t_next >= 0;
    float* g_dst = fold ? h->grad_ptr[2] : h->grad(f);
    const int* to_slot = fold ? h->tables[t_next].slot_of_pid : nullptr;
    const bool gc_out = compact_out && h->compact_F && h->all_simple_liquid && !h->has_collector;
    const int giso = (h->fiso[f] ? 1 : 0) | (h->gcompact[(f + 1) & 1] ? 2 : 0) | (gc_out ? 4 : 0);
#define LAUNCH_P2G_GRAD(G, W) hipLaunchKernelGGL((k_p2g_grad<G, W>), wgrid_pgg(h), dim3(WG), 0, h->stream, h->S, h->frame(f), h->grad(f + 1), \
                           h->grad(f), T, h->pool_idx, ggin(h, f), bcount(h, f), h->slow_dev, ag, inj, act, f, g_dst, to_slot, giso)
    if (!fuse_next) prof_begin(h, KID_P2G_GRAD);
    if (fuse_next) {
        h->stamp++;
        const BwdFuseP B = {h->frame(f - 1), h->grad(f - 1), gout(h, f - 1), h->gg_out, h->slab};
        prof_begin(h, KID_PGG_G2PG);
        if (h->all_simple_liquid)
            hipLaunchKernelGGL(k_pgg_g2pg<4>, wgrid(h), dim3(WG), 0, h->stream, h->S, h->frame(f), h->grad(f + 1), h->grad(f), T, h->pool_idx, ggin(h, f), bcount(h, f), h->slow_dev,
                               ag, inj, act, f, giso, B, grid_store(h));
        else
            hipLaunchKernelGGL((k_pgg_g2pg<3, true>), wgrid(h), dim3(WG), 0, h->stream, h->S, h->frame(f), h->grad(f + 1), h->grad(f), T, h->pool_idx, ggin(h, f), bcount(h, f), h->slow_dev,
                               ag, inj, act, f, 0, B, grid_store(h));
    } else if (h->all_simple_liquid) {
        if (h->p2g_grad_waves >= 4) LAUNCH_P2G_GRAD(false, 4);
        else if (h->p2g_grad_waves == 3) LAUNCH_P2G_GRAD(false, 3);
        else LAUNCH_P2G_GRAD(false, 2);
    } else LAUNCH_P2G_GRAD(true, 1);
    prof_end(h);
    if (fold) std::swap(h->grad_ptr[2], h->grad_ptr[f & 1]);
    h->gtbl[f & 1] = fold ? t_next : t;
    h->gcompact[f & 1] = gc_out;
    h->gpartial[f & 1] = fuse_next;
    return 0;
}

bool batchable(FeEngine** hs, int B) {
    if (B < 2 || B > FE_MAX_BATCH) return false;
    for (int i = 0; i < B; i++) if (!hs[i]) return false;
    for (int i = 0; i < B; i++) {
        FeEngine* h = hs[i];
        if (h->device != hs[0]->device || h->n != hs[0]->n || h->L != hs[0]->L || h->all_simple_liquid != hs[0]->all_simple_liquid ||
            h->sort_interval != hs[0]->sort_interval || h->p2g_grad_waves != hs[0]->p2g_grad_waves || h->g2p_grad_v != hs[0]->g2p_grad_v || h->S.wt != hs[0]->S.wt || !h->statics_host.empty() || h->has_mesh_effector || h->has_rigid || h->prof_fine ||
            (h->gs_cap > 0) != (hs[0]->gs_cap > 0)) return false;
        for (int j = 0; j < i; j++) if (hs[j] == h) return false;
    }
    return true;
}
inline dim3 wgrid_b(FeEngine** hs, int B) { unsigned g = 0; for (int i = 0; i < B; i++) g = std::max(g, wgrid(hs[i]).x); return dim3(g, B); }

void batch_fork(FeEngine** hs, int B) {
    (void)hipEventRecord(hs[0]->ev_batch, hs[0]->own_stream);
    for (int i = 1; i < B; i++) { (void)hipStreamWaitEvent(hs[i]->own_stream, hs[0]->ev_batch, 0); hs[i]->stream = hs[i]->own_stream; }
}
void batch_join(FeEngine** hs, int B) {
    for (int i = 1; i < B; i++) {
        (void)hipEventRecord(hs[i]->ev_batch, hs[i]->own_stream);
        (void)hipStreamWaitEvent(hs[0]->own_stream, hs[i]->ev_batch, 0);
        hs[i]->stream = hs[0]->own_stream;
    }
}

int substep_fwd_batch(FeEngine** hs, int B, int f, int f_global, int act, bool g2p_pending = false, bool defer_g2p = false) {
    FeEngine* h0 = hs[0];
    Batch<P2GArgs> bp; Batch<GridArgs> bg; Batch<G2PArgs> bq;
    const bool sorting = h0->sort_interval > 0 && f % h0->sort_interval == 0;
    if (sorting) batch_fork(hs, B);
    struct Join { FeEngine** hs; int B; bool on; ~Join() { if (on) batch_join(hs, B); } };
    {
    Join join{hs, B, sorting};
    for (int i = 0; i < B; i++) {
// ... 172 lines not shown
                       (const int*)h->tables[gt].pid, gt == ft ? (const int*)nullptr : (const int*)h->tables[ft].slot_of_pid);
    h->gcompact[f & 1] = false;
}

int check_device_errors(FeEngine* h) {
    int e = 0;
    HIPCK(h, hipMemcpyAsync(&e, h->err_dev, sizeof(int), hipMemcpyDeviceToHost, h->stream));
    HIPCK(h, hipStreamSynchronize(h->stream));
    if (e) {
        (void)hipMemsetAsync(h->err_dev, 0, sizeof(int), h->stream);
        FAIL(h, "particle stencil left the grid (p2g)");
    }
    if (h->fg_started) {
        int ge = 0;
        HIPCK(h, hipMemcpyAsync(&ge, h->fg_host.ctr + FGC_ERR * FG_LINE, sizeof(int), hipMemcpyDeviceToHost, h->stream));
        HIPCK(h, hipStreamSynchronize(h->stream));
        if (ge) {
            (void)hipMemsetAsync(h->fg_host.ctr + FGC_ERR * FG_LINE, 0, sizeof(int), h->stream);
            FAIL(h, "fused grid pass: a wait did not end (option fuse_grid = 0 runs the grid kernels as launches of their own)");
        }
    }
    return 0;
}

}

#include "fe_smoke.h"
#include "fe_mesh.h"

extern "C" {

const char* fe_backend(void) { return "hip-gfx950"; }
int fe_real_size(void) { return 4; }

FeEngine* fe_create(const FeConfig* cfg) {
    if (!cfg || cfg->struct_size != (int)sizeof(FeConfig)) { g_create_err = "FeConfig size mismatch"; return nullptr; }
    if (cfg->n_particles > 40000000) { g_create_err = "n_particles > 40M: a frame no longer fits 32-bit plane offsets"; return nullptr; }
    if (cfg->n_grid > 4092) { g_create_err = "n_grid > 4092: a work item names its block by three 10-bit coordinates"; return nullptr; }
    if (cfg->n_grid < 4 || cfg->n_grid % 4 != 0 || cfg->n_particles < 0 || cfg->max_substeps_local < 1 || cfg->n_substeps < 1) {
        g_create_err = "invalid FeConfig (n_grid must be a multiple of 4)"; return nullptr;
    }
    int ndev = 0;
    if (hipGetDeviceCount(&ndev) != hipSuccess || ndev == 0) { g_create_err = "no HIP device visible: the MI355X engine has no CPU fallback"; return nullptr; }
    if (cfg->device < 0 || cfg->device >= ndev) { g_create_err = "HIP device ordinal out of range"; return nullptr; }
    FeEngine* h = new FeEngine();
    if (const char* e = std::getenv("FE_SORT_INTERVAL")) h->sort_interval = std::atoi(e);
    if (const char* e = std::getenv("FE_QUAD_MIN_UNITS")) h->quad_min_units = std::atoi(e);
    if (const char* e = std::getenv("FE_G2P_GRAD_V")) h->g2p_grad_v = std::atoi(e) == 2 ? 2 : 3;
    if (const char* e = std::getenv("FE_FUSE_BWD")) h->fuse_bwd = std::atoi(e);
    if (const char* e = std::getenv("FE_FUSE_G2P")) h->fuse_g2p = std::atoi(e) != 0;
    if (const char* e = std::getenv("FE_FUSE_GRID")) h->fuse_grid = std::atoi(e);
    const char* env_lsplit = std::getenv("FE_LANE_SPLIT");
    h->cfg = *cfg; h->N = cfg->n_particles; h->L = cfg->max_substeps_local; h->n = cfg->n_grid; h->nb = cfg->n_grid / 4;
    h->Np = ((h->N + 63) / 64) * 64; if (h->Np == 0) h->Np = 64;
    h->device = cfg->device;
    auto fail = [&](const std::string& m) { g_create_err = m.empty() ? h->err : m; fe_destroy(h); return (FeEngine*)nullptr; };
    if (hipSetDevice(h->device) != hipSuccess) return fail("hipSetDevice failed");
    if (hipStreamCreateWithFlags(&h->stream, hipStreamNonBlocking) != hipSuccess) return fail("hipStreamCreate failed");
    {
        int cus = 0;
        if (hipDeviceGetAttribute(&cus, hipDeviceAttributeMultiprocessorCount, h->device) == hipSuccess && cus > 0) { h->n_cus = cus; h->quad_fit = 4 * cus; h->wgrid_cap = 4 * cus; h->wgrid_cap_pgg = 8 * cus; h->wgrid_cap_g2p = 6 * cus; }
    }
    h->own_stream = h->stream;
    SimP& S = h->S;
    S.xcd = 16;
    S.uni = 0; S.fg_base = 0; S.fg_nowait = 0;
    S.wsort = 1;
    S.lsplit = env_lsplit ? std::atoi(env_lsplit) : 3;
    S.wt = 5;
    S.N = h->N; S.Np = h->Np; S.n = h->n; S.nb = h->nb; S.ncell = h->nb * h->nb * h->nb * 64;
    S.dx = 1.0f / (float)h->n; S.inv_dx = (float)h->n; S.dt = cfg->dt;
    S.stress_scale = -cfg->dt * cfg->p_vol * 4.f * S.inv_dx * S.inv_dx;
    for (int i = 0; i < 3; i++) S.g[i] = cfg->gravity[i];
    S.bnd = to_boundary(cfg->boundary);
    h->frame_stride = (size_t)FR_WORDS * h->Np;
    const size_t ncell = (size_t)h->nb * h->nb * h->nb * 64;
    if (dev_alloc(h, &h->frames, h->frame_stride * (h->L + 2))) return fail("");
    h->frame_ptr.resize(h->L + 2);
    for (int i = 0; i < h->L + 2; i++) h->frame_ptr[i] = h->frames + (size_t)i * h->frame_stride;
    if (dev_alloc(h, &h->grads, 3 * h->grad_words())) return fail("");
    for (int i = 0; i < 3; i++) h->grad_ptr[i] = h->grads + (size_t)i * h->grad_words();
    h->tbl_of_frame.assign(h->L + 1, 0);
    h->fiso.assign(h->L + 2, 0);
    {
        const size_t nblk = (size_t)h->nb * h->nb * h->nb;
        h->items_cap = (nblk < (size_t)h->Np ? nblk : (size_t)h->Np) + (size_t)h->Np / 64 + 2;
        h->units_cap = h->items_cap + (size_t)h->Np / WG + 16 + 1024;
        if (h->items_cap * (size_t)SLAB_N * 16 >= ((size_t)1 << 31)) return fail("grid / particle count too large: the slab buffer no longer fits 32-bit byte offsets");
        if (dev_alloc(h, &h->sort_key, h->Np) || dev_alloc(h, &h->sort_rank, h->Np) || dev_alloc(h, &h->sort_cnt, ncell + 1) ||
            dev_alloc(h, &h->sort_start, ncell + 1) || dev_alloc(h, &h->sort_bcnt, ((nblk + 1 + SORT_BLK_WG - 1) / SORT_BLK_WG) * SORT_BLK_WG) || dev_alloc(h, &h->sort_partial, ((nblk + 1 + SORT_BLK_WG - 1) / SORT_BLK_WG) * PART_STRIDE) || dev_alloc(h, &h->sort_base, ((nblk + 1 + SORT_BLK_WG - 1) / SORT_BLK_WG) * SORT_BLK_WG) || dev_alloc(h, &h->sort_nact, 4)       || dev_alloc(h, &h->sort_pid, h->Np) ||
            dev_alloc(h, &h->slow_dev, 1) || dev_alloc(h, &h->frame_slow_dev, 1) || dev_alloc(h, &h->slab, h->items_cap * SLAB_N, false)) return fail("");
    }
    if (dev_alloc(h, &h->effs_dev, FE_MAX_EFF)) return fail("");
    {
        const size_t nblk = (size_t)h->nb * h->nb * h->nb;
        size_t cap = nblk;
        size_t budget_gib = 64;
        if (const char* e = std::getenv("FE_GRID_STORE_GIB")) { const long v = std::atol(e); if (v >= 0 && v <= 256) budget_gib = (size_t)v; }
        while (cap > 0 && (size_t)(h->L + 1) * cap * (GS_BLK * 16) > (budget_gib << 30)) cap /= 2;
        while (cap * (size_t)(GS_BLK * 16) >= ((size_t)1 << 31)) cap /= 2;
        h->gs_cap = (int)cap;
        if (cap > 0 && (dev_alloc(h, &h->gstore, (size_t)(h->L + 1) * cap * GS_BLK, false) || dev_alloc(h, &h->gs_flag, h->L + 1) ||
                        dev_alloc(h, &h->gs_live, (size_t)(h->L + 1) * cap))) return fail("");
        if (dev_alloc(h, &h->ent_touched, nblk) || dev_alloc(h, &h->ent_dirty, nblk) || dev_alloc(h, &h->cur_live, nblk)) return fail("");
    }
    if (dev_alloc(h, &h->pinfo, h->Np) || dev_alloc(h, &h->pool_idx, h->Np)) return fail("");
    if (ensure_table(h, 0)) return fail("");
    if (dev_alloc(h, &h->g_in, 4 * ncell) || dev_alloc(h, &h->g_out, 2 * ncell) || dev_alloc(h, &h->gg_out, 3 * ncell) || dev_alloc(h, &h->gg_in, 2 * ncell)) return fail("");
    if (dev_alloc(h, &h->blk_flag, ncell / 64) || dev_alloc(h, &h->blk_list, ncell / 64) || dev_alloc(h, &h->blk_count, 2) || dev_alloc(h, &h->err_dev, 1)) return fail("");
    {
        const size_t nblk = ncell / 64;
        if (dev_alloc(h, &h->fg_host.late, 4 * ncell) || dev_alloc(h, &h->fg_host.late_flag, nblk) || dev_alloc(h, &h->fg_host.late_list, nblk) ||
            dev_alloc(h, &h->fg_host.skipm, nblk) || dev_alloc(h, &h->fg_host.ctr, FGC_N * FG_LINE) || dev_alloc(h, &h->fg_dev, 1)) return fail("");
        if (hipMemcpyOnStream(h, h->fg_dev, &h->fg_host, sizeof(FgDev), hipMemcpyHostToDevice) != hipSuccess) return fail("hipMemcpy failed");
    }
    if (dev_alloc(h, &h->stage_r, (size_t)24 * h->Np) || dev_alloc(h, &h->stage_i, h->Np)) return fail("");
    if (dev_alloc(h, &h->node_mark, ncell) || dev_alloc(h, &h->counters, 4)) return fail("");
    {
        std::vector<int> id(h->Np);
        for (int i = 0; i < h->Np; i++) id[i] = i < h->N ? i : 0;
        if (hipMemcpyOnStream(h, h->tables[0].pid, id.data(), sizeof(int) * h->Np, hipMemcpyHostToDevice) != hipSuccess) return fail("hipMemcpy failed");
        if (hipMemcpyOnStream(h, h->tables[0].slot_of_pid, id.data(), sizeof(int) * h->Np, hipMemcpyHostToDevice) != hipSuccess) return fail("hipMemcpy failed");
    }
    if (hipEventCreate(&h->ev_t0) != hipSuccess || hipEventCreate(&h->ev_t1) != hipSuccess ||
        hipEventCreateWithFlags(&h->ev_batch, hipEventDisableTiming) != hipSuccess) return fail("hipEventCreate failed");
    if (hipStreamSynchronize(h->stream) != hipSuccess) return fail("device initialisation failed");
    return h;
}

void fe_destroy(FeEngine* h) {
    if (!h) return;
    (void)hipSetDevice(h->device);
    if (h->stream) (void)hipStreamSynchronize(h->stream);
    smoke_destroy(h);
    for (auto& t : h->tables) { if (t.info && t.info != h->pinfo) (void)hipFree(t.info);
        for (void* q : {(void*)t.pairs, (void*)t.singles, (void*)t.pid, (void*)t.items, (void*)t.meta, (void*)t.blk_first, (void*)t.active, (void*)t.blk_slot, (void*)t.slot_of_pid, (void*)t.units, (void*)t.units_p, (void*)t.nbr, (void*)t.arrive}) if (q) (void)hipFree(q); }
    void* ptrs[] = {h->frames, h->grads, h->sort_key, h->sort_rank, h->sort_cnt, h->sort_start, h->sort_bcnt, h->sort_partial, h->sort_base, h->sort_nact, h->sort_pid, h->slow_dev, h->frame_slow_dev, h->gstore, h->gs_flag, h->gs_live, h->ent_touched, h->ent_dirty, h->cur_live, h->slab, h->effs_dev, h->pinfo, h->pool_idx, h->g_in, h->g_out, h->gg_out, h->gg_in,
                    h->blk_flag, h->blk_list, h->blk_count, h->err_dev, h->stage_r, h->stage_i, h->node_mark, h->counters,
                    h->fg_host.late, h->fg_host.late_flag, h->fg_host.late_list, h->fg_host.skipm, h->fg_host.ctr, h->fg_dev,
                    h->tgt, h->chamfer, h->step_loss, h->body_start, h->body_pids, h->bodies_dev, h->statics_dev, h->collector_dev, h->hit_dev, h->hit_list, h->hit_count, h->node_work, h->node_work_count, h->pg_acc,
                    h->obs_pids, h->obs_x, h->obs_v, h->obs_u, h->sum_group, h->sum_partial, h->sum_out,
                    h->tl_step_loss, h->tl_term_loss, h->tl_terms_dev, h->tl_ref, h->tl_partial, h->tl_cnt};
    for (float* v : h->statics_vox) if (v) (void)hipFree(v);
    for (float* v : h->mesh_vox) if (v) (void)hipFree(v);
    for (void* p : ptrs) if (p) (void)hipFree(p);
    for (auto& E : h->effs) {
        void* ep[] = {E.p.pos, E.p.quat, E.p.v, E.p.w, E.p.gpos, E.p.gquat, E.p.gv, E.p.gw, E.p.abuf, E.p.gabuf, E.p.abuf_p, E.p.gabuf_p, E.p.random_vector,
                      E.p.sa, E.p.ra, E.p.gsa, E.p.gra};
        for (void* p : ep) if (p) (void)hipFree(p);
    }
    for (auto e : h->prof_ev) (void)hipEventDestroy(e);
    if (h->ev_t0) (void)hipEventDestroy(h->ev_t0);
    if (h->ev_t1) (void)hipEventDestroy(h->ev_t1);
    if (h->ev_batch) (void)hipEventDestroy(h->ev_batch);
    if (h->own_stream) (void)hipStreamDestroy(h->own_stream);
    delete h;
}

const char* fe_last_error(FeEngine* h) { return h ? h->err.c_str() : g_create_err.c_str(); }

int fe_sync(FeEngine* h) {
    FE_ENTRY(h);
    HIPCK(h, hipStreamSynchronize(h->stream));
    if (check_async(h)) return 1;
    return check_device_errors(h);
}

int fe_set_option(FeEngine* h, const char* name, double value) {
    FE_ENTRY(h);
    if (!std::strcmp(name, "sort_interval")) {
        if (value < 0) FAIL(h, "sort_interval must be >= 0");
        h->sort_interval = (int)value;
        return 0;
    }
    if (!std::strcmp(name, "item_max")) {
        if (value < 64 || value > ITEM_MAX_CAP) FAIL(h, "item_max must be in [64, 128]");
        h->item_max = (int)value;
        return 0;
    }
    if (!std::strcmp(name, "grid_store")) {
        if (value == 0) h->gs_cap = 0;
        h->gs_host_valid = false;
        return 0;
    }
    if (!std::strcmp(name, "p2g_grad_waves")) { h->p2g_grad_waves = (int)value; return 0; }
    if (!std::strcmp(name, "g2p_grad_v")) { h->g2p_grad_v = (int)value == 2 ? 2 : 3; return 0; }
    if (!std::strcmp(name, "loose_max")) { if (value < 0 || value > ITEM_MAX_CAP) FAIL(h, "loose_max must be in [0, 128]"); h->loose_max = (int)value; return 0; }
    if (!std::strcmp(name, "inject_till")) { h->inject_till = (int)value; return 0; }
    if (!std::strcmp(name, "collide_min_y")) { h->collide_min_y = (float)value; return 0; }
    if (!std::strcmp(name, "collide_type")) {
        const int t = (int)value;
        if (t < 1 || t > 3) { h->err = "collide_type must be 1 (particle), 2 (grid) or 3 (both)"; return 1; }
        h->collide_type = t; return 0;
    }
    if (!std::strcmp(name, "prof_fine")) { h->prof_fine = value != 0; return 0; }
    if (!std::strcmp(name, "xcd_map")) { if (value < 0 || value > 64) FAIL(h, "xcd_map must be 0 (none), 1 (contiguous eighths) or a run length 2..64"); h->S.xcd = (int)value; return 0; }
    if (!std::strcmp(name, "write_through")) { h->S.wt = (int)value; return 0; }
    if (!std::strcmp(name, "wave_sort")) { h->S.wsort = value != 0; return 0; }
    if (!std::strcmp(name, "lane_split")) { if (value < 0 || value > 7) FAIL(h, "lane_split is a bit set: 1 k_p2g, 2 k_g2p_grad2, 4 k_p2g_grad"); h->S.lsplit = (int)value; return 0; }
    if (!std::strcmp(name, "fold_reorder")) { h->fold_reorder = value != 0; return 0; }
    if (!std::strcmp(name, "compact_F")) { h->compact_F = value != 0; return 0; }
    if (!std::strcmp(name, "fuse_g2p")) { h->fuse_g2p = value != 0; return 0; }
    if (!std::strcmp(name, "sort_keys_in_g2p")) { h->sort_keys_in_g2p = value != 0; return 0; }
    if (!std::strcmp(name, "sort_one_scan")) { h->sort_one_scan = value != 0; return 0; }
    if (!std::strcmp(name, "fuse_bwd")) { h->fuse_bwd = (int)value; return 0; }
    if (!std::strcmp(name, "fuse_grid")) { if (value < 0 || value > 6 || ((int)value & 3) == 3) FAIL(h, "fuse_grid must be 0 (separate grid kernels), 1 (fused where nothing slow is expected) or 2 (wherever possible), + 4: never wait"); h->fuse_grid = (int)value; return 0; }
    if (!std::strcmp(name, "quad_min_units")) { h->quad_min_units = (int)value; return 0; }
    if (!std::strcmp(name, "pgg_quad_min_units")) { h->pgg_quad_min_units = (int)value; return 0; }
    if (!std::strcmp(name, "pack_units")) { if (value < 0 || value > 2) FAIL(h, "pack_units must be 0, 1 or 2"); h->pack_units = (int)value; return 0; }
    if (!std::strcmp(name, "quad_fit")) { if (value < 0) FAIL(h, "quad_fit must be >= 0"); h->quad_fit = (int)value; return 0; }
    if (!std::strcmp(name, "quad_max")) { if (value < 0 || value > QUAD_MAX) FAIL(h, "quad_max must be in [0, 64]"); h->quad = (int)value; return 0; }
    if (!std::strcmp(name, "ggrid_cap")) { if (value < 1) FAIL(h, "ggrid_cap must be >= 1"); h->ggrid_cap = (int)value; return 0; }
    if (!std::strcmp(name, "wgrid_cap_pgg")) { if (value < 64) FAIL(h, "wgrid_cap_pgg must be >= 64"); h->wgrid_cap_pgg = (int)value; return 0; }
    if (!std::strcmp(name, "wgrid_cap_g2p")) { if (value < 64) FAIL(h, "wgrid_cap_g2p must be >= 64"); h->wgrid_cap_g2p = (int)value; return 0; }
    if (!std::strcmp(name, "wgrid_cap")) { if (value < 64) { h->err = "wgrid_cap must be >= 64"; return 1; } h->wgrid_cap = (int)value; return 0; }
    if (!std::strcmp(name, "param_grad")) {
        if (value != 0 && h->has_rigid) FAIL(h, "param_grad: scenes with MAT_RIGID particles are not supported (their density also enters the shape-matching centre of mass)");
        if (value != 0 && !h->pg_acc && dev_alloc(h, &h->pg_acc, (size_t)3 * h->N)) return 1;
        h->param_grad = value != 0;
        return 0;
    }
    if (!std::strcmp(name, "task_pair_chunk")) {
        if (value < 0 || value > (1 << 30) || ((long long)value) % 64 != 0) FAIL(h, "task_pair_chunk must be 0 (chosen by the engine) or a positive multiple of 64");
        h->task_pair_chunk = (int)value;
        return 0;
    }
    if (!std::strcmp(name, "threads")) return 0;
    FAIL(h, std::string("unknown option: ") + name);
}

int fe_get_option(FeEngine* h, const char* name, double* value) {
    FE_ENTRY(h);
    if (!value) FAIL(h, "fe_get_option: null output");
    const struct { const char* n; double v; } tab[] = {
        {"sort_interval", (double)h->sort_interval}, {"item_max", (double)h->item_max}, {"grid_store", h->gs_cap > 0 ? 1.0 : 0.0},
        {"p2g_grad_waves", (double)h->p2g_grad_waves}, {"g2p_grad_v", (double)h->g2p_grad_v}, {"loose_max", (double)h->loose_max},
        {"inject_till", (double)h->inject_till}, {"collide_min_y", (double)h->collide_min_y}, {"collide_type", (double)h->collide_type},
        {"prof_fine", h->prof_fine ? 1.0 : 0.0}, {"xcd_map", (double)h->S.xcd}, {"write_through", (double)h->S.wt}, {"wave_sort", (double)h->S.wsort}, {"lane_split", (double)h->S.lsplit}, {"fold_reorder", h->fold_reorder ? 1.0 : 0.0}, {"compact_F", h->compact_F ? 1.0 : 0.0}, {"fuse_g2p", h->fuse_g2p ? 1.0 : 0.0}, {"fuse_bwd", (double)h->fuse_bwd}, {"fuse_grid", (double)h->fuse_grid}, {"sort_keys_in_g2p", (double)h->sort_keys_in_g2p}, {"sort_one_scan", (double)h->sort_one_scan},
        {"quad_min_units", (double)h->quad_min_units}, {"pgg_quad_min_units", (double)h->pgg_quad_min_units}, {"quad_max", (double)h->quad}, {"quad_fit", (double)h->quad_fit}, {"pack_units", (double)h->pack_units},
        {"wgrid_cap", (double)h->wgrid_cap}, {"wgrid_cap_g2p", (double)h->wgrid_cap_g2p}, {"wgrid_cap_pgg", (double)h->wgrid_cap_pgg}, {"ggrid_cap", (double)h->ggrid_cap}, {"param_grad", h->param_grad ? 1.0 : 0.0}, {"task_pair_chunk", (double)h->task_pair_chunk}, {"threads", 0.0}};
    for (const auto& t : tab) if (!std::strcmp(name, t.n)) { *value = t.v; return 0; }
    FAIL(h, std::string("unknown option: ") + name);
}

int fe_init_particles(FeEngine* h, const fe_real* x, const int* used, const int* mat, const int* mat_cls,
                      const fe_real* mu, const fe_real* lam, const fe_real* rho, const int* body_id) {
    FE_ENTRY(h);
    const int N = h->N;
    std::vector<float4> info(h->Np, make_float4(0, 0, 0, 0));
    std::vector<float> C0((size_t)9 * N, 0.f), F0((size_t)9 * N, 0.f), v0((size_t)3 * N, 0.f);
    h->mat_host.assign(mat, mat + N);
    bool simple = true;
    for (int i = 0; i < N; i++) {
        if (mat_cls[i] < 0 || mat_cls[i] > 0xffff || mat[i] < 0 || mat[i] > 0xffff) FAIL(h, "material id out of range");
        int bits = (mat_cls[i] & 0xffff) | ((mat[i] & 0xffff) << 16);
        float w; std::memcpy(&w, &bits, 4);
        info[i] = make_float4(mu[i], lam[i], h->cfg.p_vol * rho[i], w);
        simple = simple && mu[i] == 0.f && mat_cls[i] == FE_MAT_LIQUID;
        F0[(size_t)i * 9] = F0[(size_t)i * 9 + 4] = F0[(size_t)i * 9 + 8] = 1.f;
    }
    h->all_simple_liquid = simple;
    {
        bool uni = N > 0;
        for (int i = 1; i < N && uni; i++) uni = std::memcmp(&info[i], &info[0], sizeof(float4)) == 0;
        h->S.uni = uni ? 1 : 0;
        if (uni) { h->S.uinfo[0] = info[0].x; h->S.uinfo[1] = info[0].y; h->S.uinfo[2] = info[0].z; h->S.uinfo[3] = info[0].w; }
    }
    h->has_rigid = false; h->n_bodies = 0;
    for (int i = 0; i < N; i++) {
        const int b = body_id ? body_id[i] : 0;
        if (b < 0) FAIL(h, "negative body_id");
        if (b + 1 > h->n_bodies) h->n_bodies = b + 1;
        if (mat_cls[i] == FE_MAT_RIGID) h->has_rigid = true;
    }
    if (h->has_rigid && h->param_grad) FAIL(h, "param_grad: scenes with MAT_RIGID particles are not supported (their density also enters the shape-matching centre of mass)");
    for (void* q : {(void*)h->bodies_dev, (void*)h->body_start, (void*)h->body_pids}) if (q) (void)hipFree(q);
    h->bodies_dev = nullptr; h->body_start = nullptr; h->body_pids = nullptr;
    if (h->has_rigid) {
        std::vector<RigidBody> bodies(h->n_bodies);
        std::vector<int> cnt(h->n_bodies, 0);
        std::vector<std::vector<int>> members(h->n_bodies);
        std::memset(bodies.data(), 0, sizeof(RigidBody) * bodies.size());
        for (int i = 0; i < N; i++) {
            const int b = body_id ? body_id[i] : 0;
            if (cnt[b]++ == 0) bodies[b].rigid = mat_cls[i] == FE_MAT_RIGID;
            if (mat_cls[i] == FE_MAT_RIGID) members[b].push_back(i);
        }
        std::vector<int> start(h->n_bodies + 1, 0), pids;
        for (int b = 0; b < h->n_bodies; b++) {
            bodies[b].inv_n = cnt[b] ? 1.f / (float)cnt[b] : 0.f;
            pids.insert(pids.end(), members[b].begin(), members[b].end());
            start[b + 1] = (int)pids.size();
        }
        if (dev_alloc(h, &h->bodies_dev, h->n_bodies) || dev_alloc(h, &h->body_start, h->n_bodies + 1) || dev_alloc(h, &h->body_pids, pids.size())) return 1;
        HIPCK(h, hipMemcpyAsync(h->bodies_dev, bodies.data(), sizeof(RigidBody) * h->n_bodies, hipMemcpyHostToDevice, h->stream));
        HIPCK(h, hipMemcpyAsync(h->body_start, start.data(), sizeof(int) * start.size(), hipMemcpyHostToDevice, h->stream));
        HIPCK(h, hipMemcpyAsync(h->body_pids, pids.data(), sizeof(int) * pids.size(), hipMemcpyHostToDevice, h->stream));
        HIPCK(h, hipStreamSynchronize(h->stream));
    }
    HIPCK(h, hipMemcpyAsync(h->pinfo, info.data(), sizeof(float4) * h->Np, hipMemcpyHostToDevice, h->stream));
    HIPCK(h, hipStreamSynchronize(h->stream));
    h->tbl_of_frame[0] = 0;
    h->tail_used = true;
    h->keys_frame = -1;
    std::fill(h->fiso.begin(), h->fiso.end(), 0);
    h->gcompact[0] = h->gcompact[1] = false;
    h->gpartial[0] = h->gpartial[1] = false;
    return upload_planes(h, h->frame(0), h->pid_of(0), x, v0.data(), C0.data(), F0.data(), used, 0);
}

int fe_substep(FeEngine* h, int f, int f_global, int act) {
    FE_ENTRY(h);
    if (f < 0 || f >= h->L) FAIL(h, "substep frame out of range");
    if (substep_fwd(h, f, f_global, act)) return 1;
    return check_async(h);
}
int fe_substep_grad(FeEngine* h, int f, int f_global, int act) {
    FE_ENTRY(h);
    if (f < 0 || f >= h->L) FAIL(h, "substep frame out of range");
    if (substep_bwd(h, f, f_global, act)) return 1;
    return check_async(h);
}
int fe_step(FeEngine* h, int f0, int f_global0, int n, int act) {
    FE_ENTRY(h);
    if (f0 < 0 || f0 + n > h->L) FAIL(h, "step frames out of range");
    bool pending = false;
    for (int i = 0; i < n; i++) {
        const bool defer = i + 1 < n && fusable_fwd(h, f0 + i + 1);
        if (substep_fwd(h, f0 + i, f_global0 + i, act, pending, defer)) return 1;
        pending = defer;
    }
    return check_async(h);
}
int fe_step_grad(FeEngine* h, int f0, int f_global0, int n, int act) {
    FE_ENTRY(h);
    if (f0 < 0 || f0 + n > h->L) FAIL(h, "step frames out of range");
    bool done = false;
    if (n > 1 && fetch_gs_flags(h)) return 1;
    for (int i = n - 1; i >= 0; i--) {
        const bool fuse = i > 0 && fusable_bwd(h, f0 + i);
        if (substep_bwd(h, f0 + i, f_global0 + i, act, f0 + i > 0 ? f0 + i - 1 : -1, i > 0, done, fuse)) return 1;
        done = fuse;
    }
    return check_async(h);
}
int fe_step_batch(FeEngine** hs, int n_env, int f0, int f_global0, int n, int act) {
    if (!hs || n_env < 1) return 1;
    for (int e = 0; e < n_env; e++) if (!hs[e]) return 1;
    FeEngine* h = hs[0];
    FE_ENTRY(h);
    if (!batchable(hs, n_env)) {
        for (int e = 0; e < n_env; e++) if (fe_step(hs[e], f0, f_global0, n, act)) { h->err = hs[e]->err; return 1; }
        return 0;
    }
    if (f0 < 0 || f0 + n > h->L) FAIL(h, "step frames out of range");
    BatchStreams bs(hs, n_env);
    bool pending = false;
    for (int i = 0; i < n; i++) {
        bool defer = i + 1 < n;
        for (int e = 0; e < n_env && defer; e++) defer = fusable_fwd(hs[e], f0 + i + 1);
        if (substep_fwd_batch(hs, n_env, f0 + i, f_global0 + i, act, pending, defer)) { for (int e = 1; e < n_env; e++) if (!hs[e]->err.empty()) h->err = hs[e]->err; return 1; }
        pending = defer;
    }
    return check_async(h);
}
int fe_step_grad_batch(FeEngine** hs, int n_env, int f0, int f_global0, int n, int act) {
    if (!hs || n_env < 1) return 1;
    for (int e = 0; e < n_env; e++) if (!hs[e]) return 1;
    FeEngine* h = hs[0];
    FE_ENTRY(h);
    for (int e = 0; e < n_env; e++) if (hs[e]->param_grad) FAIL(h, "option param_grad is not available in batched backward passes (fe_step_grad_batch): step the engine on its own");
    if (!batchable(hs, n_env)) {
        for (int e = 0; e < n_env; e++) if (fe_step_grad(hs[e], f0, f_global0, n, act)) { h->err = hs[e]->err; return 1; }
        return 0;
    }
    if (f0 < 0 || f0 + n > h->L) FAIL(h, "step frames out of range");
    BatchStreams bs(hs, n_env);
    bool done = false;
    if (n > 1) for (int e = 0; e < n_env; e++) if (fetch_gs_flags(hs[e])) { h->err = hs[e]->err; return 1; }
    for (int i = n - 1; i >= 0; i--) {
        bool fuse = i > 0;
        for (int e = 0; e < n_env && fuse; e++) fuse = hs[e]->all_simple_liquid && fusable_bwd(hs[e], f0 + i);
        if (substep_bwd_batch(hs, n_env, f0 + i, f_global0 + i, act, done, fuse)) { for (int e = 1; e < n_env; e++) if (!hs[e]->err.empty()) h->err = hs[e]->err; return 1; }
        done = fuse;
    }
    return check_async(h);
}

int fe_get_frame(FeEngine* h, int f, fe_real* x, fe_real* v, fe_real* C, fe_real* F, int* used) {
    FE_ENTRY(h);
    CHECK_FRAME(h, f);
    if (F) full_F_of_frame(h, f);
    if (download_planes(h, h->frame(f), h->pid_of(f), x, v, C, F, used)) return 1;
    return check_device_errors(h);
}
int fe_set_frame(FeEngine* h, int f, const fe_real* x, const fe_real* v, const fe_real* C, const fe_real* F, const int* used) {
    FE_ENTRY(h);
    CHECK_FRAME(h, f);
    if (f == h->keys_frame) h->keys_frame = -1;
    h->tail_used = true;
    h->gs_host_valid = false;
    if (h->gs_cap > 0) HIPCK(h, hipMemsetAsync(h->gs_flag + f, 0, sizeof(int), h->stream));
    if (F) h->fiso[f] = 0;
    return upload_planes(h, h->frame(f), h->pid_of(f), x, v, C, F, used, 0);
}
int fe_get_frame_dev(FeEngine* h, int f, fe_real* x, fe_real* v, fe_real* C, fe_real* F, int* used) {
    FE_ENTRY(h);
    CHECK_FRAME(h, f);
    const int mask = (x ? 1 : 0) | (v ? 2 : 0) | (C ? 4 : 0) | (F ? 8 : 0) | (used ? 16 : 0);
    if (!mask || h->N == 0) return 0;
    if (F) full_F_of_frame(h, f);
    hipLaunchKernelGGL(k_unpack, pgrid(h), dim3(256), 0, h->stream, h->N, (size_t)h->Np, h->frame(f), h->pid_of(f), x, v, C, F, used, mask);
    HIPCK(h, hipStreamSynchronize(h->stream));
    return check_device_errors(h);
}
int fe_set_frame_dev(FeEngine* h, int f, const fe_real* x, const fe_real* v, const fe_real* C, const fe_real* F, const int* used) {
    FE_ENTRY(h);
    CHECK_FRAME(h, f);
    if (f == h->keys_frame) h->keys_frame = -1;
    h->tail_used = true;
    h->gs_host_valid = false;
    if (h->gs_cap > 0) HIPCK(h, hipMemsetAsync(h->gs_flag + f, 0, sizeof(int), h->stream));
    const int mask = (x ? 1 : 0) | (v ? 2 : 0) | (C ? 4 : 0) | (F ? 8 : 0) | (used ? 16 : 0);
    if (!mask || h->N == 0) return 0;
    if (F) h->fiso[f] = 0;
    hipLaunchKernelGGL(k_pack, pgrid(h), dim3(256), 0, h->stream, h->N, (size_t)h->Np, h->frame(f), h->pid_of(f), x, v, C, F, used, mask, 0);
    HIPCK(h, hipStreamSynchronize(h->stream));
    return check_async(h);
}
int fe_copy_frame(FeEngine* h, int src, int dst) {
    FE_ENTRY(h);
    CHECK_FRAME(h, src); CHECK_FRAME(h, dst);
    if (src == dst) return 0;
    HIPCK(h, hipMemcpyAsync(h->frame(dst), h->frame(src), sizeof(float) * h->frame_stride, hipMemcpyDeviceToDevice, h->stream));
    h->tbl_of_frame[dst] = h->tbl_of_frame[src];
    h->fiso[dst] = h->fiso[src];
    h->tail_used = true;
    if (dst == h->keys_frame) h->keys_frame = -1;
    if (src == h->keys_frame) h->keys_frame = dst;
    h->gs_host_valid = false;
    if (h->gs_cap > 0) HIPCK(h, hipMemsetAsync(h->gs_flag + dst, 0, sizeof(int), h->stream));
    return 0;
}
int fe_copy_grad(FeEngine* h, int src, int dst) {
    FE_ENTRY(h);
    CHECK_FRAME(h, src); CHECK_FRAME(h, dst);
    if (h->gpartial[src & 1]) FAIL(h, "this frame's adjoint was passed on in registers inside a fused fe_step_grad call and is not in memory (after fe_step_grad(f0, n) only the adjoint of frame f0 is defined; option fuse_bwd = 0 keeps every frame's)");
    if ((src & 1) != (dst & 1)) {
        HIPCK(h, hipMemcpyAsync(h->grad(dst), h->grad(src), sizeof(float) * GR_WORDS * h->Np, hipMemcpyDeviceToDevice, h->stream));
        h->gtbl[dst & 1] = h->gtbl[src & 1];
        h->gcompact[dst & 1] = h->gcompact[src & 1];
        h->gpartial[dst & 1] = false;
    }
    if (src != dst) {
        FrameV s = frame_view(h->frame(src), h->Np), d = frame_view(h->frame(dst), h->Np);
        HIPCK(h, hipMemcpyAsync(d.used.ptr(), s.used.ptr(), sizeof(int) * h->Np, hipMemcpyDeviceToDevice, h->stream));
    }
    return 0;
}
int fe_reset_grad(FeEngine* h) {
    FE_ENTRY(h);
    if (smoke_reset_grad_impl(h)) return 1;
    HIPCK(h, hipMemsetAsync(h->grad_ptr[0], 0, sizeof(float) * h->grad_words(), h->stream));
    HIPCK(h, hipMemsetAsync(h->grad_ptr[1], 0, sizeof(float) * h->grad_words(), h->stream));
    h->gtbl[0] = h->gtbl[1] = -1;
    h->gcompact[0] = h->gcompact[1] = false;
    h->gpartial[0] = h->gpartial[1] = false;
    if (h->pg_acc) HIPCK(h, hipMemsetAsync(h->pg_acc, 0, sizeof(double) * 3 * (size_t)h->N, h->stream));
    for (auto& E : h->effs) {
        const int Fm = h->L + 1, ad = E.p.action_dim > 0 ? E.p.action_dim : 1;
        HIPCK(h, hipMemsetAsync(E.p.gpos, 0, sizeof(float) * 3 * Fm, h->stream));
        HIPCK(h, hipMemsetAsync(E.p.gquat, 0, sizeof(float) * 4 * Fm, h->stream));
        HIPCK(h, hipMemsetAsync(E.p.gv, 0, sizeof(float) * 3 * Fm, h->stream));
        HIPCK(h, hipMemsetAsync(E.p.gw, 0, sizeof(float) * 3 * Fm, h->stream));
        HIPCK(h, hipMemsetAsync(E.p.gsa, 0, sizeof(float) * Fm, h->stream));
        HIPCK(h, hipMemsetAsync(E.p.gra, 0, sizeof(float) * Fm, h->stream));
        HIPCK(h, hipMemsetAsync(E.p.gabuf, 0, sizeof(float) * (size_t)h->cfg.max_action_steps * ad, h->stream));
        HIPCK(h, hipMemsetAsync(E.p.gabuf_p, 0, sizeof(float) * ad, h->stream));
    }
    return 0;
}
int fe_reset_grad_till_frame(FeEngine* h, int f) {
    FE_ENTRY(h);
    CHECK_FRAME(h, f);
    return 0;
}
int fe_agent_set_collector(FeEngine* h, const FeBoundary* b, int mat) {
    FE_ENTRY(h);
    (void)hipSetDevice(h->device);
    h->has_collector = b != nullptr;
    h->collector_mat = mat;
    if (!b) return 0;
    const BoundaryP p = to_boundary(*b);
    if (!h->collector_dev && dev_alloc(h, &h->collector_dev, 1)) return 1;
    if (hipMemcpyOnStream(h, h->collector_dev, &p, sizeof(BoundaryP), hipMemcpyHostToDevice) != hipSuccess) { h->err = "hipMemcpy failed"; return 1; }
    return 0;
}
int fe_agent_reset_grad_till_frame(FeEngine* h, int f) {
    FE_ENTRY(h);
    CHECK_FRAME(h, f);
    for (auto& E : h->effs) {
        if (f == 0) break;
        HIPCK(h, hipMemsetAsync(E.p.gpos, 0, sizeof(float) * 3 * f, h->stream));
// ... 264 lines not shown
    h->loss_steps = max_loss_steps;
    if (dev_alloc(h, &h->tgt, (size_t)max_loss_steps * h->N * 3) || dev_alloc(h, &h->chamfer, max_loss_steps) || dev_alloc(h, &h->step_loss, max_loss_steps)) return 1;
    return 0;
}
int fe_loss_set_target(FeEngine* h, int s, const fe_real* x) {
    FE_ENTRY(h);
    if (s < 0 || s >= h->loss_steps) FAIL(h, "loss step out of range");
    HIPCK(h, hipMemcpyAsync(h->tgt + (size_t)s * h->N * 3, x, sizeof(float) * 3 * h->N, hipMemcpyHostToDevice, h->stream));
    HIPCK(h, hipStreamSynchronize(h->stream));
    return 0;
}
int fe_loss_clear(FeEngine* h) {
    FE_ENTRY(h);
    if (!h->loss_steps) return 0;
    HIPCK(h, hipMemsetAsync(h->chamfer, 0, sizeof(float) * h->loss_steps, h->stream));
    HIPCK(h, hipMemsetAsync(h->step_loss, 0, sizeof(float) * h->loss_steps, h->stream));
    return 0;
}
int fe_loss_step(FeEngine* h, int s, int f, int matching_mat, fe_real weight) {
    FE_ENTRY(h);
    if (s < 0 || s >= h->loss_steps) FAIL(h, "loss step out of range");
    CHECK_FRAME(h, f);
    hipLaunchKernelGGL(k_loss_fwd, pgrid(h), dim3(256), 0, h->stream, h->S, h->frame(f), h->pid_of(f), h->pinfo,
                       h->tgt + (size_t)s * h->N * 3, matching_mat, h->chamfer + s);
    hipLaunchKernelGGL(k_loss_sum, dim3(1), dim3(64), 0, h->stream, h->chamfer + s, h->step_loss + s, weight);
    return check_async(h);
}
int fe_loss_step_grad(FeEngine* h, int s, int f, int matching_mat, fe_real weight, fe_real step_loss_grad) {
    FE_ENTRY(h);
    if (s < 0 || s >= h->loss_steps) FAIL(h, "loss step out of range");
    CHECK_FRAME(h, f);
    if (h->gpartial[f & 1]) FAIL(h, "this frame's adjoint was passed on in registers inside a fused fe_step_grad call and is not in memory (after fe_step_grad(f0, n) only the adjoint of frame f0 is defined; option fuse_bwd = 0 keeps every frame's)");
    const int gt = grad_table_for_frame(h, f), ft = h->tbl_of_frame[f];
    hipLaunchKernelGGL(k_loss_bwd, pgrid(h), dim3(256), 0, h->stream, h->S, h->frame(f), h->grad(f), h->tables[gt].pid, gt == ft ? (const int*)nullptr : h->tables[ft].slot_of_pid, h->pinfo,
                       h->tgt + (size_t)s * h->N * 3, matching_mat, weight * step_loss_grad);
    return check_async(h);
}
int fe_loss_get(FeEngine* h, fe_real* step_loss, int n) {
    FE_ENTRY(h);
    if (n > h->loss_steps) FAIL(h, "loss_get: n too large");
    HIPCK(h, hipMemcpyAsync(step_loss, h->step_loss, sizeof(float) * n, hipMemcpyDeviceToHost, h->stream));
    HIPCK(h, hipStreamSynchronize(h->stream));
    return 0;
}

int fe_mesh_sdf(int device, const float* verts, int nv, const int* faces, int nf, const float* points, long long n_points, float* sdf) {
    if (nv <= 0 || nf <= 0 || n_points < 0 || !verts || !faces || (n_points > 0 && (!points || !sdf))) { g_create_err = "fe_mesh_sdf: invalid arguments"; return 1; }
    for (long long i = 0; i < (long long)nf * 3; i++) if (faces[i] < 0 || faces[i] >= nv) { g_create_err = "fe_mesh_sdf: face index out of range"; return 1; }
    if (n_points == 0) return 0;
    int ndev = 0;
    if (hipGetDeviceCount(&ndev) != hipSuccess || ndev == 0) { g_create_err = "no HIP device visible: the MI355X engine has no CPU fallback"; return 1; }
    if (device < 0 || device >= ndev || hipSetDevice(device) != hipSuccess) { g_create_err = "HIP device ordinal out of range"; return 1; }
    float *dv = nullptr, *dp = nullptr, *ds = nullptr; int* df = nullptr;
    auto done = [&](int rc, const char* msg) { if (msg) g_create_err = msg; (void)hipFree(dv); (void)hipFree(df); (void)hipFree(dp); (void)hipFree(ds); return rc; };
    if (hipMalloc(&dv, sizeof(float) * 3 * nv) != hipSuccess || hipMalloc(&df, sizeof(int) * 3 * nf) != hipSuccess ||
        hipMalloc(&dp, sizeof(float) * 3 * n_points) != hipSuccess || hipMalloc(&ds, sizeof(float) * n_points) != hipSuccess)
        return done(1, "fe_mesh_sdf: hipMalloc failed");
    if (hipMemcpy(dv, verts, sizeof(float) * 3 * nv, hipMemcpyHostToDevice) != hipSuccess || hipMemcpy(df, faces, sizeof(int) * 3 * nf, hipMemcpyHostToDevice) != hipSuccess ||
        hipMemcpy(dp, points, sizeof(float) * 3 * n_points, hipMemcpyHostToDevice) != hipSuccess)
        return done(1, "fe_mesh_sdf: upload failed");
    hipLaunchKernelGGL(k_mesh_sdf, dim3((unsigned)((n_points + 255) / 256)), dim3(256), 0, 0, dv, df, nf, dp, n_points, ds);
    if (hipGetLastError() != hipSuccess || hipDeviceSynchronize() != hipSuccess) return done(1, "fe_mesh_sdf: kernel failed");
    if (hipMemcpy(sdf, ds, sizeof(float) * n_points, hipMemcpyDeviceToHost) != hipSuccess) return done(1, "fe_mesh_sdf: download failed");
    return done(0, nullptr);
}

int fe_get_stats(FeEngine* h, int f, FeStats* out) {
    FE_ENTRY(h);
    CHECK_FRAME(h, f);
    const int ncell = h->nb * h->nb * h->nb * 64;
    HIPCK(h, hipMemsetAsync(h->counters, 0, sizeof(unsigned long long) * 4, h->stream));
    hipLaunchKernelGGL(k_stats_mark, pgrid(h), dim3(256), 0, h->stream, h->S, h->frame(f), h->node_mark, h->counters);
    hipLaunchKernelGGL(k_stats_count, dim3((ncell + 255) / 256), dim3(256), 0, h->stream, ncell, h->node_mark, h->counters);
    unsigned long long c[4];
    int slow = 0;
    HIPCK(h, hipMemcpyAsync(c, h->counters, sizeof(c), hipMemcpyDeviceToHost, h->stream));
    HIPCK(h, hipMemcpyAsync(&slow, h->slow_dev, sizeof(int), hipMemcpyDeviceToHost, h->stream));
    HIPCK(h, hipMemsetAsync(h->slow_dev, 0, sizeof(int), h->stream));
    HIPCK(h, hipStreamSynchronize(h->stream));
    out->n_used = (long long)c[0]; out->n_cells_touched = (long long)c[1]; out->n_blocks_active = (long long)c[2];
    out->n_slow_path = slow; out->bytes_state = (long long)h->bytes;
    return check_async(h);
}
int fe_get_work_stats(FeEngine* h, int f, long long out[FE_WORK_STATS]) { return fe_get_work_stats_n(h, f, out, FE_WORK_STATS); }
int fe_get_work_stats_n(FeEngine* h, int f, long long* out_, int n_out) {
    FE_ENTRY(h);
    CHECK_FRAME(h, f);
    if (!out_ || n_out < 0) FAIL(h, "fe_get_work_stats_n: bad output buffer");
    long long out[FE_WORK_STATS];
    struct Copy { long long* src; long long* dst; int n; ~Copy() { for (int i = 0; i < n && i < FE_WORK_STATS; i++) dst[i] = src[i]; } } copy_out{out, out_, n_out};
    for (int i = 0; i < 24; i++) out[i] = 0;
    const int t = h->tbl_of_frame[f];
    if (t < 0 || t >= (int)h->tables.size() || !h->tables[t].meta) return 0;
    int meta[16];
    HIPCK(h, hipMemcpyAsync(meta, h->tables[t].meta, sizeof(meta), hipMemcpyDeviceToHost, h->stream));
    HIPCK(h, hipStreamSynchronize(h->stream));
    for (int i = 0; i < 5; i++) out[i] = meta[i];
    out[3] += meta[11] + meta[12];
    out[4] += meta[8]; out[14] = meta[8]; out[15] = meta[10];
    out[13] = meta[7] - meta[1];
    out[16] = meta[14]; out[17] = meta[15]; out[18] = meta[13]; out[19] = meta[11]; out[20] = meta[12];
    std::vector<int4> items((size_t)std::max(meta[0], 0));
    if (!items.empty()) {
        HIPCK(h, hipMemcpyAsync(items.data(), h->tables[t].items, sizeof(int4) * items.size(), hipMemcpyDeviceToHost, h->stream));
        HIPCK(h, hipStreamSynchronize(h->stream));
    }
    int last_block = -1;
    for (const int4& it : items) {
        const int c = it.z;
        const int b = c <= 1 ? 0 : c <= 4 ? 1 : c <= 8 ? 2 : c <= 16 ? 3 : c <= 32 ? 4 : c <= 64 ? 5 : 6;
        out[5 + b]++;
        if (it.x != last_block) { out[12]++; last_block = it.x; }
        if (h->S.lsplit) {
            for (int w0 = 0; w0 < c; w0 += 64) { const int cnt = std::min(64, c - w0); if (cnt <= FE_SPLIT9_MAX) out[21]++; else if (cnt <= FE_SPLIT3_MAX) out[22]++; }
        }
    }
    return check_async(h);
}
#ifdef FE_TIMELINE
int fe_timeline_read(FeEngine* h, int kid, unsigned long long* out) {
    FE_ENTRY(h);
    if (kid < 0 || kid >= KID_COUNT || !h->tl_dev) FAIL(h, "no timeline");
    HIPCK(h, hipMemcpyAsync(out, h->tl_dev + (size_t)kid * TL_WGS * 9, sizeof(unsigned long long) * TL_WGS * 9, hipMemcpyDeviceToHost, h->stream));
    HIPCK(h, hipStreamSynchronize(h->stream));
    return 0;
}
#endif
static int param_grad_copy(FeEngine* h, double* g_mu, double* g_lam, double* g_rho, hipMemcpyKind kind) {
    if (!h->pg_acc) FAIL(h, "param_grad is not enabled: fe_set_option(h, \"param_grad\", 1) first");
    double* dst[3] = {g_mu, g_lam, g_rho};
    for (int i = 0; i < 3; i++)
        if (dst[i]) HIPCK(h, hipMemcpyAsync(dst[i], h->pg_acc + (size_t)i * h->N, sizeof(double) * h->N, kind, h->stream));
    HIPCK(h, hipStreamSynchronize(h->stream));
    return check_async(h);
}
int fe_param_grad_get(FeEngine* h, double* g_mu, double* g_lam, double* g_rho) { FE_ENTRY(h); return param_grad_copy(h, g_mu, g_lam, g_rho, hipMemcpyDeviceToHost); }
int fe_param_grad_get_dev(FeEngine* h, double* g_mu, double* g_lam, double* g_rho) { FE_ENTRY(h); return param_grad_copy(h, g_mu, g_lam, g_rho, hipMemcpyDeviceToDevice); }
int fe_param_grad_reset(FeEngine* h) {
    FE_ENTRY(h);
    if (!h->pg_acc) FAIL(h, "param_grad is not enabled: fe_set_option(h, \"param_grad\", 1) first");
    HIPCK(h, hipMemsetAsync(h->pg_acc, 0, sizeof(double) * 3 * (size_t)h->N, h->stream));
    return 0;
}

int fe_obs_set_particles(FeEngine* h, const int* pids, int n) {
    FE_ENTRY(h);
    if (n < 0) FAIL(h, "fe_obs_set_particles: n < 0");
    int *d_p = nullptr, *d_u = nullptr; float *d_x = nullptr, *d_v = nullptr;
    if (pids && n > 0) {
        for (int i = 0; i < n; i++) if (pids[i] < 0 || pids[i] >= h->N) FAIL(h, "fe_obs_set_particles: particle id out of range (the list is unchanged)");
        if (dev_alloc(h, &d_p, (size_t)n, false) || dev_alloc(h, &d_x, (size_t)3 * n) || dev_alloc(h, &d_v, (size_t)3 * n) || dev_alloc(h, &d_u, (size_t)n)) {
            for (void* q : {(void*)d_p, (void*)d_x, (void*)d_v, (void*)d_u}) if (q) (void)hipFree(q);
            return 1;
        }
        if (hipMemcpyOnStream(h, d_p, pids, sizeof(int) * (size_t)n, hipMemcpyHostToDevice) != hipSuccess) {
            for (void* q : {(void*)d_p, (void*)d_x, (void*)d_v, (void*)d_u}) (void)hipFree(q);
            FAIL(h, "fe_obs_set_particles: hipMemcpy failed");
        }
    } else n = 0;
    HIPCK(h, hipStreamSynchronize(h->stream));
    for (void* q : {(void*)h->obs_pids, (void*)h->obs_x, (void*)h->obs_v, (void*)h->obs_u}) if (q) (void)hipFree(q);
    h->obs_pids = d_p; h->obs_x = d_x; h->obs_v = d_v; h->obs_u = d_u; h->obs_n = n;
    return 0;
}
static int obs_gather(FeEngine* h, int f, float* x, float* v, int* used) {
    const int n = h->obs_n;
    hipLaunchKernelGGL(k_obs_gather, dim3((n + 255) / 256), dim3(256), 0, h->stream, n, h->N, (size_t)h->Np, h->frame(f), (const int*)h->tables[h->tbl_of_frame[f]].slot_of_pid,
                       (const int*)h->obs_pids, x, v, used);
    return 0;
}
int fe_obs_get(FeEngine* h, int f, fe_real* x, fe_real* v, int* used) {
    FE_ENTRY(h);
    CHECK_FRAME(h, f);
    if (!h->obs_pids) FAIL(h, "no observation list: fe_obs_set_particles first");
// ... 265 lines not shown
```

### include/fluidengine.h

```cpp
#ifndef FLUIDENGINE_H
#define FLUIDENGINE_H

#ifdef __cplusplus
extern "C" {
#endif

#ifndef FE_REAL
#define FE_REAL float
#endif
typedef FE_REAL fe_real;

typedef struct FeEngine FeEngine;

enum {
    FE_MAT_LIQUID              = 200,
    FE_MAT_PLASTO_ELASTIC      = 201,
    FE_MAT_ELASTIC             = 202,
    FE_MAT_RIGID               = 203,
    FE_MAT_PLASTO_ELASTIC_DEMO = 204
};

enum { FE_BOUNDARY_CUBE = 0, FE_BOUNDARY_CYLINDER = 1 };

typedef struct FeBoundary {
// ... 66 lines not shown
                     const fe_real* F, const int* used);
int fe_copy_frame(FeEngine* h, int src, int dst);
int fe_copy_grad(FeEngine* h, int src, int dst);
int fe_reset_grad(FeEngine* h);
int fe_reset_grad_till_frame(FeEngine* h, int f);
int fe_get_grad(FeEngine* h, int f, fe_real* gx, fe_real* gv, fe_real* gC, fe_real* gF);
int fe_add_grad(FeEngine* h, int f, const fe_real* gx, const fe_real* gv, const fe_real* gC,
                const fe_real* gF);
int fe_add_grad_dev(FeEngine* h, int f, const fe_real* gx, const fe_real* gv, const fe_real* gC,
                    const fe_real* gF);
int fe_get_mat(FeEngine* h, int* mat);

int fe_add_effector(FeEngine* h, const FeEffectorDesc* desc, const fe_real* random_vector);
int fe_eff_set_act_range(FeEngine* h, int e, const int* act_range, int n);
int fe_eff_get_state(FeEngine* h, int e, int f, fe_real* state8);
int fe_eff_set_state(FeEngine* h, int e, int f, const fe_real* state8);
int fe_eff_get_vw(FeEngine* h, int e, int f, fe_real* v3, fe_real* w3);
int fe_eff_set_vw(FeEngine* h, int e, int f, const fe_real* v3, const fe_real* w3);
int fe_eff_get_sr(FeEngine* h, int e, int f, fe_real* s, fe_real* r);
int fe_eff_set_sr(FeEngine* h, int e, int f, fe_real s, fe_real r);
int fe_eff_set_action(FeEngine* h, int e, int s, int s_global, int n_substeps,
                      const fe_real* action);
int fe_eff_set_action_grad(FeEngine* h, int e, int s, int s_global, int n_substeps);
int fe_eff_apply_action_p(FeEngine* h, int e, const fe_real* action_p);
int fe_eff_apply_action_p_grad(FeEngine* h, int e);
int fe_eff_get_action_grad(FeEngine* h, int e, int s, int n, fe_real* grad);
int fe_agent_copy_frame(FeEngine* h, int src, int dst);
int fe_agent_copy_grad(FeEngine* h, int src, int dst);
int fe_agent_reset_grad_till_frame(FeEngine* h, int f);
int fe_agent_set_collector(FeEngine* h, const FeBoundary* b, int mat);

typedef struct FeSdfDesc {
    int     struct_size;
    int     res;
    fe_real T_mesh_to_voxels[16];
    fe_real friction;
    fe_real softness;
} FeSdfDesc;
int fe_add_static(FeEngine* h, const FeSdfDesc* desc, const fe_real* voxels);
int fe_eff_set_mesh(FeEngine* h, int e, const FeSdfDesc* desc, const fe_real* voxels);

typedef struct FeSmokeConfig {
    int     struct_size;
    int     res;
    int     solver_iters;
    int     q_dim;
    int     max_steps_local;
    fe_real dt;
    fe_real decay;
    fe_real high_T, low_T;
    int     lower_y, higher_y;
} FeSmokeConfig;
int fe_smoke_create(FeEngine* h, const FeSmokeConfig* cfg);
int fe_smoke_step(FeEngine* h, int s, int f);
int fe_smoke_step_grad(FeEngine* h, int s, int f);
int fe_smoke_get_frame(FeEngine* h, int s, fe_real* v, fe_real* v_tmp, fe_real* div, fe_real* p, fe_real* q);
int fe_smoke_set_frame(FeEngine* h, int s, const fe_real* v, const fe_real* v_tmp, const fe_real* div, const fe_real* p, const fe_real* q);
int fe_smoke_get_grad(FeEngine* h, int s, fe_real* gv, fe_real* gq);
int fe_smoke_add_grad(FeEngine* h, int s, const fe_real* gv, const fe_real* gq);
int fe_smoke_copy_frame(FeEngine* h, int src, int dst);
int fe_smoke_copy_grad(FeEngine* h, int src, int dst);
int fe_smoke_reset_grad(FeEngine* h);
int fe_smoke_reset_grad_till_frame(FeEngine* h, int s);

int fe_loss_alloc(FeEngine* h, int max_loss_steps);
int fe_loss_set_target(FeEngine* h, int s, const fe_real* x);
int fe_loss_clear(FeEngine* h);
int fe_loss_step(FeEngine* h, int s, int f, int matching_mat, fe_real weight);
int fe_loss_step_grad(FeEngine* h, int s, int f, int matching_mat, fe_real weight,
                      fe_real step_loss_grad);
int fe_loss_get(FeEngine* h, fe_real* step_loss, int n);

int fe_mesh_sdf(int device, const float* verts, int nv, const int* faces, int nf,
                const float* points, long long n_points, float* sdf);

typedef struct FeStats {
    long long n_used;
    long long n_cells_touched;
    long long n_blocks_active;
    long long n_slow_path;
    long long bytes_state;
} FeStats;
int fe_get_stats(FeEngine* h, int f, FeStats* out);
#define FE_WORK_STATS 24
int fe_get_work_stats_n(FeEngine* h, int f, long long* out, int n);
int fe_get_work_stats(FeEngine* h, int f, long long out[FE_WORK_STATS]);
int    fe_timer_start(FeEngine* h);
double fe_timer_stop_ms(FeEngine* h);
int fe_profile_enable(FeEngine* h, int on);
int fe_profile_read(FeEngine* h, char* buf, int buf_len, double* ms_total, long long* launches, int cap);

#ifdef __cplusplus
}
#endif
#endif
```

Measured before the change: 11450 substep_pairs/s.

## Size grid-kernel launches from active-block counts published to mapped host memory

The sort kernels now write the active-block count, tagged with a serial, into host-mapped pinned memory. The host reads it when launching the grid update kernels and sizes the workgroup count to the active list, with a margin when it falls back to a lagged count from an earlier sort. It can exceed the old fixed cap of 1024 workgroups, up to a configurable limit. This replaces a fixed grid that could be too small or too large for the active block list, at the cost of a system-scope atomic store and a host-side lookup on every launch. A gravity add is also turned into an fmaf.

```diff
diff --git a/__graft_entry__.py b/__graft_entry__.py
--- a/__graft_entry__.py
+++ b/__graft_entry__.py
@@ -25,7 +25,7 @@
 
 
 def build(force=False):
-    srcs = [os.path.join(CSRC, f) for f in ('fe_engine.hip', 'fe_math.h', 'fe_smoke.h', 'fe_mesh.h', 'fe_param_grad.h', 'fe_summary.h', 'fe_task_loss.h')] + \
+    srcs = [os.path.join(CSRC, f) for f in ('fe_engine.hip', 'fe_math.h', 'fe_grid_launch.h', 'fe_smoke.h', 'fe_mesh.h', 'fe_param_grad.h', 'fe_summary.h', 'fe_task_loss.h')] + \
            [os.path.join(ROOT, 'include', f) for f in ('fluidengine.h', 'fluidengine_ext.h')]
     stamp, want = HIP_LIB + '.srchash', _source_hash(srcs)
     have = open(stamp).read().strip() if os.path.exists(stamp) else ''
diff --git a/fluidlab_amd/_capi.py b/fluidlab_amd/_capi.py
--- a/fluidlab_amd/_capi.py
+++ b/fluidlab_amd/_capi.py
@@ -259,7 +259,7 @@
         self._ck(self.lib.fe_set_option(self.h, name.encode(), float(value)))
 
     OPTION_NAMES = ('sort_interval', 'item_max', 'grid_store', 'p2g_grad_waves', 'g2p_grad_v', 'loose_max', 'xcd_map', 'write_through',
-                    'wave_sort', 'lane_split', 'fold_reorder', 'compact_F', 'fuse_g2p', 'fuse_bwd', 'quad_min_units', 'pgg_quad_min_units', 'quad_max', 'quad_fit', 'pack_units', 'wgrid_cap', 'wgrid_cap_g2p', 'wgrid_cap_pgg', 'ggrid_cap', 'collide_type')
+                    'wave_sort', 'lane_split', 'fold_reorder', 'compact_F', 'fuse_g2p', 'fuse_bwd', 'quad_min_units', 'pgg_quad_min_units', 'quad_max', 'quad_fit', 'pack_units', 'wgrid_cap', 'wgrid_cap_g2p', 'wgrid_cap_pgg', 'ggrid_cap', 'grid_list_launch', 'grid_hint', 'grid_hint_margin', 'grid_one_cap', 'collide_type')
 
     def get_option(self, name):
         v = C.c_double(0.0)
@@ -669,10 +669,11 @@
         self._ck(self.lib.fe_get_stats(self.h, int(f), C.byref(st)))
         return {k: getattr(st, k) for k, _ in FeStats._fields_}
 
-    def get_work_stats(self, f):
-        out = (C.c_longlong * 24)()
+    def get_work_stats(self, f, launches=False):
+        out = (C.c_longlong * 30)()
+        out[24] = out[27] = -1
         if hasattr(self.lib, 'fe_get_work_stats_n'):
-            self._ck(self.lib.fe_get_work_stats_n(self.h, int(f), out, 24))
+            self._ck(self.lib.fe_get_work_stats_n(self.h, int(f), out, 30))
         else:
             self._ck(self.lib.fe_get_work_stats(self.h, int(f), out))
         keys = ('n_items', 'tail_start', 'n_active_blocks', 'n_multi_item_workgroups', 'n_single_item_blocks')
@@ -686,6 +687,10 @@
         d['packed'] = bool(out[18])
         d['n_leftover_items'] = int(out[19]) + int(out[20])
         d['n_split9_waves'], d['n_split3_waves'] = int(out[21]), int(out[22])
+        if launches:
+            kinds = ('none', 'lagged', 'exact', 'forced')
+            d['grid_launch'] = {'wgs': int(out[23]), 'hint': int(out[24]), 'kind': kinds[int(out[25]) & 3]}
+            d['grid_grad_launch'] = {'wgs': int(out[26]), 'hint': int(out[27]), 'kind': kinds[int(out[28]) & 3]}
         return d
 
     def timer_start(self):
diff --git a/fluidlab_amd/csrc/fe_engine.hip b/fluidlab_amd/csrc/fe_engine.hip
--- a/fluidlab_amd/csrc/fe_engine.hip
+++ b/fluidlab_amd/csrc/fe_engine.hip
@@ -10,6 +10,7 @@
 #include "../../include/fluidengine.h"
 #include "../../include/fluidengine_ext.h"
 #include "fe_math.h"
+#include "fe_grid_launch.h"
 
 static_assert(sizeof(fe_real) == 4, "the HIP engine is fp32 (macros.py:207-211)");
 
@@ -1187,9 +1188,9 @@
                                               float (*trace)[3] = nullptr, const AgentP* agent = nullptr, int f = 0, float* vdyn = nullptr,
                                               bool* dyn_hit = nullptr) {
     float inv = 1.f / gi.w;
-    vo[0] = inv * gi.x + S.dt * S.g[0];
-    vo[1] = inv * gi.y + S.dt * S.g[1];
-    vo[2] = inv * gi.z + S.dt * S.g[2];
+    vo[0] = fmaf(S.dt, S.g[0], inv * gi.x);
+    vo[1] = fmaf(S.dt, S.g[1], inv * gi.y);
+    vo[2] = fmaf(S.dt, S.g[2], inv * gi.z);
     float xn[3] = {(float)i * S.dx, (float)j * S.dx, (float)k * S.dx};
     if (STATICS) {
 #pragma unroll
@@ -3055,9 +3056,13 @@
     }
     __syncthreads();
 }
+struct ListLenOut { unsigned long long* word; unsigned serial; };
+__device__ __forceinline__ void list_len_out(const ListLenOut& LL, int n_act) {
+    if (LL.word) __hip_atomic_store(LL.word, ((unsigned long long)LL.serial << 32) | (unsigned)n_act, __ATOMIC_RELAXED, __HIP_MEMORY_SCOPE_SYSTEM);
+}
 template <bool ONE>
 __device__ __forceinline__ bool sort_side_jobs(int nblk, int nb, const int* __restrict__ bcnt, int blk_wgs, int scan_wgs, int* cnt, int* start, int* nact, int* active, int* blk_slot,
-                                               int* act_done, int act_target, int* meta) {
+                                               int* act_done, int act_target, int* meta, ListLenOut LL) {
     const int lane = threadIdx.x & 63;
     if ((int)blockIdx.x >= blk_wgs + scan_wgs) {
         const int b = (blockIdx.x - blk_wgs - scan_wgs) * 256 + threadIdx.x;
@@ -3090,8 +3095,11 @@
         if (!on && b < nblk) blk_slot[b] = -1;
         if (ONE) {
             __syncthreads();
-            if (threadIdx.x == 0 && __hip_atomic_fetch_add(act_done, 1, __ATOMIC_RELAXED, __HIP_MEMORY_SCOPE_AGENT) == act_target - 1)
-                meta[2] = __hip_atomic_load(nact, __ATOMIC_RELAXED, __HIP_MEMORY_SCOPE_AGENT);
+            if (threadIdx.x == 0 && __hip_atomic_fetch_add(act_done, 1, __ATOMIC_RELAXED, __HIP_MEMORY_SCOPE_AGENT) == act_target - 1) {
+                const int n_act = __hip_atomic_load(nact, __ATOMIC_RELAXED, __HIP_MEMORY_SCOPE_AGENT);
+                meta[2] = n_act;
+                list_len_out(LL, n_act);
+            }
         }
         return true;
     }
@@ -3125,7 +3133,7 @@
 __global__ __launch_bounds__(256) void k_sort_blk_partial(int nblk, int nb, int ITEM_MAX, int loose_max, int quad_max, const int* __restrict__ bcnt, int* partial,
                                                           int blk_wgs, int scan_wgs, int* cnt, int* start, int* nact, int* active, int* blk_slot) {
     __shared__ int sh[4][NSUM];
-    if (sort_side_jobs<false>(nblk, nb, bcnt, blk_wgs, scan_wgs, cnt, start, nact, active, blk_slot, nullptr, 0, nullptr)) return;
+    if (sort_side_jobs<false>(nblk, nb, bcnt, blk_wgs, scan_wgs, cnt, start, nact, active, blk_slot, nullptr, 0, nullptr, ListLenOut{nullptr, 0u})) return;
     int n[4], ex[NSUM], tot[NSUM];
     const BlkSums m = blk_sums4(blk_ask4(bcnt), nblk, ITEM_MAX, loose_max, quad_max, n);
     wg_scan6(m, sh, ex, tot);
@@ -3133,7 +3141,7 @@
     for (int k = 0; k < NSUM; k++) if ((int)threadIdx.x == k) partial[blockIdx.x * PART_STRIDE + k] = tot[k];
 }
 __device__ __forceinline__ void sort_blk_final_body(int (*sh)[NSUM], const int4 n4, const BlkSums& pb, const BlkSums& pa, int nblk, int nb, int ncell, int ITEM_MAX, int loose_max, int quad_max,
-                                                    int* cnt, int* start, int4* items, int2* pairs, int* singles, int* singles_c, int2* blk_first, int* blk_base, const int* __restrict__ nact, int* meta) {
+                                                    int* cnt, int* start, int4* items, int2* pairs, int* singles, int* singles_c, int2* blk_first, int* blk_base, const int* __restrict__ nact, int* meta, ListLenOut LL) {
     const int tid = threadIdx.x;
     int n[4], ex[NSUM], tot[NSUM];
     const BlkSums m = blk_sums4(n4, nblk, ITEM_MAX, loose_max, quad_max, n);
@@ -3141,7 +3149,7 @@
     wg_scan6(pb, sh, exb, before);
     wg_scan6(pa, sh, exa, total);
     wg_scan6(m, sh, ex, tot);
-    if (blockIdx.x == 0 && tid == 0) { meta[0] = total[2]; meta[1] = total[0]; if (nact) meta[2] = *nact; meta[3] = total[3]; meta[4] = total[4]; meta[6] = total[5]; meta[7] = total[0] + total[1]; meta[8] = total[6] + total[9] + total[10];
+    if (blockIdx.x == 0 && tid == 0) { meta[0] = total[2]; meta[1] = total[0]; if (nact) { const int n_act = *nact; meta[2] = n_act; list_len_out(LL, n_act); } meta[3] = total[3]; meta[4] = total[4]; meta[6] = total[5]; meta[7] = total[0] + total[1]; meta[8] = total[6] + total[9] + total[10];
                                        meta[11] = total[7]; meta[12] = total[8]; }
     const int b0 = blockIdx.x * SORT_BLK_WG + tid * 4;
     if (b0 > nblk) return;
@@ -3184,7 +3192,7 @@
     else for (int u = 0; u < 4; u++) if (b0 + u < nblk) blk_first[b0 + u] = bf[u];
 }
 __global__ __launch_bounds__(256) void k_sort_blk_final(int nblk, int nb, int ncell, int ITEM_MAX, int loose_max, int quad_max, const int* __restrict__ bcnt, int* cnt, int* start,
-                                                        const int* __restrict__ partial, int4* items, int2* pairs, int* singles, int* singles_c, int2* blk_first, int* blk_base, const int* __restrict__ nact, int* meta) {
+                                                        const int* __restrict__ partial, int4* items, int2* pairs, int* singles, int* singles_c, int2* blk_first, int* blk_base, const int* __restrict__ nact, int* meta, ListLenOut LL) {
     __shared__ int sh[4][NSUM];
     const int tid = threadIdx.x;
     const int4 n4 = blk_ask4(bcnt);
@@ -3193,14 +3201,14 @@
 #pragma unroll
         for (int k = 0; k < NSUM; k++) { const int t = partial[w * PART_STRIDE + k]; pa.v[k] += t; if (w < (int)blockIdx.x) pb.v[k] += t; }
     }
-    sort_blk_final_body(sh, n4, pb, pa, nblk, nb, ncell, ITEM_MAX, loose_max, quad_max, cnt, start, items, pairs, singles, singles_c, blk_first, blk_base, nact, meta);
-}
-struct SortScanSync { int* ready; int ready_target; int* act_done; int act_target; };
+    sort_blk_final_body(sh, n4, pb, pa, nblk, nb, ncell, ITEM_MAX, loose_max, quad_max, cnt, start, items, pairs, singles, singles_c, blk_first, blk_base, nact, meta, LL);
+}
+struct SortScanSync { int* ready; int ready_target; int* act_done; int act_target; ListLenOut LL; };
 __global__ __launch_bounds__(256) void k_sort_blk_scan(int nblk, int nb, int ncell, int ITEM_MAX, int loose_max, int quad_max, const int* __restrict__ bcnt, int* partial, int blk_wgs, int scan_wgs,
                                                        int* cnt, int* start, int* nact, int* active, int* blk_slot, int4* items, int2* pairs, int* singles, int* singles_c, int2* blk_first,
                                                        int* blk_base, int* meta, SortScanSync Y) {
     __shared__ int sh[4][NSUM];
-    if (sort_side_jobs<true>(nblk, nb, bcnt, blk_wgs, scan_wgs, cnt, start, nact, active, blk_slot, Y.act_done, Y.act_target, meta)) return;
+    if (sort_side_jobs<true>(nblk, nb, bcnt, blk_wgs, scan_wgs, cnt, start, nact, active, blk_slot, Y.act_done, Y.act_target, meta, Y.LL)) return;
     const int tid = threadIdx.x;
     const int4 n4 = blk_ask4(bcnt);
     {
@@ -3222,7 +3230,7 @@
 #pragma unroll
         for (int k = 0; k < NSUM; k++) { const int t = __hip_atomic_load(partial + w * PART_STRIDE + k, __ATOMIC_RELAXED, __HIP_MEMORY_SCOPE_AGENT); pa.v[k] += t; if (w < (int)blockIdx.x) pb.v[k] += t; }
     }
-    sort_blk_final_body(sh, n4, pb, pa, nblk, nb, ncell, ITEM_MAX, loose_max, quad_max, cnt, start, items, pairs, singles, singles_c, blk_first, blk_base, nullptr, meta);
+    sort_blk_final_body(sh, n4, pb, pa, nblk, nb, ncell, ITEM_MAX, loose_max, quad_max, cnt, start, items, pairs, singles, singles_c, blk_first, blk_base, nullptr, meta, ListLenOut{nullptr, 0u});
 }
 
 struct UnitLists { int nF, tB, lB, lS, tS; };
@@ -3777,7 +3785,17 @@
     unsigned char* hit_dev = nullptr;
     int* hit_list = nullptr; int* hit_count = nullptr;
     NodeWork* node_work = nullptr; int* node_work_count = nullptr;
-    int ggrid_cap = 1024;
+    int ggrid_cap = 0;
+    int grid_list_launch = 1;
+    int grid_hint_force = -1;
+    int grid_one_cap = FE_GL_ONE_CAP_WGS;
+    int grid_hint_margin = FE_GL_MARGIN_PCT;
+    unsigned long long* len_host = nullptr; unsigned long long* len_dev = nullptr; size_t len_slots = 0;
+    std::vector<unsigned> tbl_serial;
+    unsigned sort_serial = 0, hint_floor_serial = 0;
+    struct SortRef { int t; unsigned serial; }; SortRef sort_ring[32]; unsigned sort_ring_n = 0;
+    struct GridLaunchRec { int wgs = 0, hint = -1, kind = 0; };
+    std::vector<GridLaunchRec> gl_fwd, gl_bwd;
     bool fold_reorder = true;
     int wgrid_cap_pgg = 2048;
     int wgrid_cap_g2p = 2048;
@@ -3877,7 +3895,31 @@
 inline dim3 wgrid(FeEngine* h) { int g = (h->N + 63) / 64 + 8; if (g < 512) g = 512; return dim3(g < h->wgrid_cap ? g : h->wgrid_cap); }
 inline dim3 wgrid_g2p(FeEngine* h) { int g = (h->N + 63) / 64 + 8; if (g < 512) g = 512; return dim3(g < h->wgrid_cap_g2p ? g : h->wgrid_cap_g2p); }
 inline dim3 wgrid_pgg(FeEngine* h) { int g = (h->N + 63) / 64 + 8; if (g < 512) g = 512; return dim3(g < h->wgrid_cap_pgg ? g : h->wgrid_cap_pgg); }
-inline dim3 ggrid(FeEngine* h) { int blocks = h->nb * h->nb * h->nb; int g = (blocks + 3) / 4; return dim3(g < h->ggrid_cap ? g : h->ggrid_cap); }
+inline dim3 ggrid(FeEngine* h) { return dim3(fe_grid_launch_fixed(h->nb * h->nb * h->nb, h->ggrid_cap)); }
+inline dim3 ggrid_list(FeEngine* h, int t, int f, bool fwd) {
+    const int blocks = h->nb * h->nb * h->nb;
+    long long hint = -1; int kind = FE_GL_NONE;
+    if (h->grid_list_launch) {
+        if (h->grid_hint_force >= 0) { hint = h->grid_hint_force; kind = FE_GL_FORCED; }
+        else if (h->len_host && t > 0 && (size_t)t < h->len_slots) {
+            const unsigned mine = h->tbl_serial[t];
+            const unsigned long long w = __atomic_load_n(h->len_host + t, __ATOMIC_RELAXED);
+            if (mine != 0u && mine > h->hint_floor_serial && (unsigned)(w >> 32) == mine) { hint = (long long)(unsigned)w; kind = FE_GL_EXACT; }
+            else if (fwd) {
+                for (unsigned i = 0; i < 32u && i < h->sort_ring_n; i++) {
+                    const FeEngine::SortRef& r = h->sort_ring[(h->sort_ring_n - 1u - i) % 32u];
+                    if (r.serial <= h->hint_floor_serial) break;
+                    const unsigned long long v = __atomic_load_n(h->len_host + r.t, __ATOMIC_RELAXED);
+                    if ((unsigned)(v >> 32) == r.serial) { hint = (long long)(unsigned)v; kind = FE_GL_LAGGED; break; }
+                }
+            }
+        }
+    }
+    const int g = fe_grid_launch_wgs(hint, h->grid_hint_margin, kind != FE_GL_LAGGED, blocks, h->ggrid_cap, h->grid_one_cap);
+    FeEngine::GridLaunchRec& rec = (fwd ? h->gl_fwd : h->gl_bwd)[f];
+    rec.wgs = g; rec.hint = (int)hint; rec.kind = kind;
+    return dim3(g);
+}
 
 void prof_drain(FeEngine* h);
 void prof_begin(FeEngine* h, int kid) {
@@ -4004,9 +4046,16 @@
                        tn.active, tn.meta, tn.blk_slot, h->sort_nact);
     if (fine) { prof_end(h); prof_begin(h, KID_SORT_SCAN); }
     const int blk_wgs = (nblk + 1 + SORT_BLK_WG - 1) / SORT_BLK_WG, scan_wgs = (nblk + 63) / 64, act_wgs = (nblk + 255) / 256;
+    ListLenOut LL = {nullptr, 0u};
+    if ((size_t)id_new < h->len_slots) {
+        if (++h->sort_serial == 0u) { h->sort_serial = 1u; h->hint_floor_serial = 0u; std::fill(h->tbl_serial.begin(), h->tbl_serial.end(), 0u); h->sort_ring_n = 0; }
+        h->tbl_serial[id_new] = h->sort_serial;
+        h->sort_ring[h->sort_ring_n++ % 32] = {id_new, h->sort_serial};
+        LL = {h->len_dev + id_new, h->sort_serial};
+    }
     if (h->sort_one_scan && blk_wgs <= 2 * h->n_cus) {
         h->scan_ready += blk_wgs; h->scan_act += act_wgs;
-        const SortScanSync Y = {h->sort_nact + 1, h->scan_ready, h->sort_nact + 2, h->scan_act};
+        const SortScanSync Y = {h->sort_nact + 1, h->scan_ready, h->sort_nact + 2, h->scan_act, LL};
         hipLaunchKernelGGL(k_sort_blk_scan, dim3(blk_wgs + scan_wgs + act_wgs), dim3(256), 0, h->stream, nblk, h->nb, ncell, h->item_max, h->loose_max, quad_max(h), h->sort_bcnt, h->sort_partial,
                            blk_wgs, scan_wgs, h->sort_cnt, h->sort_start, h->sort_nact, tn.active, tn.blk_slot, tn.items, tn.pairs, tn.singles, tn.singles + h->items_cap, tn.blk_first,
                            h->sort_base, tn.meta, Y);
@@ -4014,7 +4063,7 @@
         hipLaunchKernelGGL(k_sort_blk_partial, dim3(blk_wgs + scan_wgs + act_wgs), dim3(256), 0, h->stream, nblk, h->nb, h->item_max, h->loose_max, quad_max(h), h->sort_bcnt, h->sort_partial,
                            blk_wgs, scan_wgs, h->sort_cnt, h->sort_start, h->sort_nact, tn.active, tn.blk_slot);
         hipLaunchKernelGGL(k_sort_blk_final, dim3(blk_wgs), dim3(256), 0, h->stream, nblk, h->nb, ncell, h->item_max, h->loose_max, quad_max(h), h->sort_bcnt, h->sort_cnt, h->sort_start, h->sort_partial,
-                           tn.items, tn.pairs, tn.singles, tn.singles + h->items_cap, tn.blk_first, h->sort_base, h->sort_nact, tn.meta);
+                           tn.items, tn.pairs, tn.singles, tn.singles + h->items_cap, tn.blk_first, h->sort_base, h->sort_nact, tn.meta, LL);
     }
     if (fine) { prof_end(h); prof_begin(h, KID_SORT_PERM); }
     int* pid_dst = id_old == id_new ? h->sort_pid : tn.pid;
@@ -4051,7 +4100,8 @@
 
 template <bool KEEP>
 void launch_grid(FeEngine* h, const TableP& T, int f, const AgentP& ag) {
-#define LAUNCH_GRID(ST_, DY_) hipLaunchKernelGGL(HIP_KERNEL_NAME(k_grid<KEEP, ST_, DY_>), ggrid(h), dim3(256), 0, h->stream, h->S, T, h->slab, h->g_in, gout(h, f), \
+    const dim3 gg = ggrid_list(h, h->tbl_of_frame[f], f, !KEEP);
+#define LAUNCH_GRID(ST_, DY_) hipLaunchKernelGGL(HIP_KERNEL_NAME(k_grid<KEEP, ST_, DY_>), gg, dim3(256), 0, h->stream, h->S, T, h->slab, h->g_in, gout(h, f), \
                            h->blk_list, bcount(h, f), h->blk_flag, grid_store(h), f, h->frame_slow_dev, statics_p(h), ag)
     if (grid_collide(h)) { if (h->statics_host.empty()) LAUNCH_GRID(false, true); else LAUNCH_GRID(true, true); }
     else { if (h->statics_host.empty()) LAUNCH_GRID(false, false); else LAUNCH_GRID(true, false); }
@@ -4203,7 +4253,8 @@
     prof_end(h);
     }
     prof_begin(h, KID_GRID_GRAD);
-#define LAUNCH_GRID_GRAD(ST_, DY_) hipLaunchKernelGGL(HIP_KERNEL_NAME(k_grid_grad<ST_, DY_>), ggrid(h), dim3(256), 0, h->stream, h->S, T, h->slab, h->g_in, h->gg_out, \
+    const dim3 ggg = ggrid_list(h, t, f, false);
+#define LAUNCH_GRID_GRAD(ST_, DY_) hipLaunchKernelGGL(HIP_KERNEL_NAME(k_grid_grad<ST_, DY_>), ggg, dim3(256), 0, h->stream, h->S, T, h->slab, h->g_in, h->gg_out, \
                            ggin(h, f), h->blk_list, bcount(h, f), h->blk_flag, grid_store(h), f, statics_p(h), ag, h->node_work, h->node_work_count)
     if (grid_collide(h)) {
         if (!h->node_work && (dev_alloc(h, &h->node_work, (size_t)h->S.ncell, false) || dev_alloc(h, &h->node_work_count, 1))) return 1;
@@ -4542,6 +4593,14 @@
     for (int i = 0; i < 3; i++) h->grad_ptr[i] = h->grads + (size_t)i * h->grad_words();
     h->tbl_of_frame.assign(h->L + 1, 0);
     h->fiso.assign(h->L + 2, 0);
+    h->gl_fwd.assign(h->L + 1, FeEngine::GridLaunchRec()); h->gl_bwd.assign(h->L + 1, FeEngine::GridLaunchRec());
+    {
+        h->len_slots = 2 * (size_t)(h->L + 1) + 1;
+        if (hipHostMalloc((void**)&h->len_host, sizeof(unsigned long long) * h->len_slots, hipHostMallocMapped) != hipSuccess ||
+            hipHostGetDevicePointer((void**)&h->len_dev, h->len_host, 0) != hipSuccess) return fail("hipHostMalloc (list lengths) failed");
+        std::memset(h->len_host, 0, sizeof(unsigned long long) * h->len_slots);
+        h->tbl_serial.assign(h->len_slots, 0u);
+    }
     {
         const size_t nblk = (size_t)h->nb * h->nb * h->nb;
         h->items_cap = (nblk < (size_t)h->Np ? nblk : (size_t)h->Np) + (size_t)h->Np / 64 + 2;
@@ -4614,6 +4673,7 @@
     if (h->ev_t1) (void)hipEventDestroy(h->ev_t1);
     if (h->ev_batch) (void)hipEventDestroy(h->ev_batch);
     if (h->own_stream) (void)hipStreamDestroy(h->own_stream);
+    if (h->len_host) (void)hipHostFree(h->len_host);
     delete h;
 }
 
@@ -4670,7 +4730,11 @@
     if (!std::strcmp(name, "pack_units")) { if (value < 0 || value > 2) FAIL(h, "pack_units must be 0, 1 or 2"); h->pack_units = (int)value; return 0; }
     if (!std::strcmp(name, "quad_fit")) { if (value < 0) FAIL(h, "quad_fit must be >= 0"); h->quad_fit = (int)value; return 0; }
     if (!std::strcmp(name, "quad_max")) { if (value < 0 || value > QUAD_MAX) FAIL(h, "quad_max must be in [0, 64]"); h->quad = (int)value; return 0; }
-    if (!std::strcmp(name, "ggrid_cap")) { if (value < 1) FAIL(h, "ggrid_cap must be >= 1"); h->ggrid_cap = (int)value; return 0; }
+    if (!std::strcmp(name, "ggrid_cap")) { if (value < 0) FAIL(h, "ggrid_cap must be >= 1 (a hard upper bound on the grid kernels' workgroups) or 0 (derived)"); h->ggrid_cap = (int)value; return 0; }
+    if (!std::strcmp(name, "grid_list_launch")) { h->grid_list_launch = value != 0.0 ? 1 : 0; return 0; }
+    if (!std::strcmp(name, "grid_hint")) { h->grid_hint_force = value < 0 ? -1 : (int)value; return 0; }
+    if (!std::strcmp(name, "grid_one_cap")) { if (value < 1) FAIL(h, "grid_one_cap must be >= 1"); h->grid_one_cap = (int)value; return 0; }
+    if (!std::strcmp(name, "grid_hint_margin")) { if (value < 100 || value > 400) FAIL(h, "grid_hint_margin is a percentage in [100, 400]"); h->grid_hint_margin = (int)value; return 0; }
     if (!std::strcmp(name, "wgrid_cap_pgg")) { if (value < 64) FAIL(h, "wgrid_cap_pgg must be >= 64"); h->wgrid_cap_pgg = (int)value; return 0; }
     if (!std::strcmp(name, "wgrid_cap_g2p")) { if (value < 64) FAIL(h, "wgrid_cap_g2p must be >= 64"); h->wgrid_cap_g2p = (int)value; return 0; }
     if (!std::strcmp(name, "wgrid_cap")) { if (value < 64) { h->err = "wgrid_cap must be >= 64"; return 1; } h->wgrid_cap = (int)value; return 0; }
@@ -4698,7 +4762,7 @@
         {"inject_till", (double)h->inject_till}, {"collide_min_y", (double)h->collide_min_y}, {"collide_type", (double)h->collide_type},
         {"prof_fine", h->prof_fine ? 1.0 : 0.0}, {"xcd_map", (double)h->S.xcd}, {"write_through", (double)h->S.wt}, {"wave_sort", (double)h->S.wsort}, {"lane_split", (double)h->S.lsplit}, {"fold_reorder", h->fold_reorder ? 1.0 : 0.0}, {"compact_F", h->compact_F ? 1.0 : 0.0}, {"fuse_g2p", h->fuse_g2p ? 1.0 : 0.0}, {"fuse_bwd", (double)h->fuse_bwd}, {"fuse_grid", (double)h->fuse_grid}, {"sort_keys_in_g2p", (double)h->sort_keys_in_g2p}, {"sort_one_scan", (double)h->sort_one_scan},
         {"quad_min_units", (double)h->quad_min_units}, {"pgg_quad_min_units", (double)h->pgg_quad_min_units}, {"quad_max", (double)h->quad}, {"quad_fit", (double)h->quad_fit}, {"pack_units", (double)h->pack_units},
-        {"wgrid_cap", (double)h->wgrid_cap}, {"wgrid_cap_g2p", (double)h->wgrid_cap_g2p}, {"wgrid_cap_pgg", (double)h->wgrid_cap_pgg}, {"ggrid_cap", (double)h->ggrid_cap}, {"param_grad", h->param_grad ? 1.0 : 0.0}, {"task_pair_chunk", (double)h->task_pair_chunk}, {"threads", 0.0}};
+        {"wgrid_cap", (double)h->wgrid_cap}, {"wgrid_cap_g2p", (double)h->wgrid_cap_g2p}, {"wgrid_cap_pgg", (double)h->wgrid_cap_pgg}, {"ggrid_cap", (double)h->ggrid_cap}, {"grid_list_launch", (double)h->grid_list_launch}, {"grid_hint", (double)h->grid_hint_force}, {"grid_hint_margin", (double)h->grid_hint_margin}, {"grid_one_cap", (double)h->grid_one_cap}, {"param_grad", h->param_grad ? 1.0 : 0.0}, {"task_pair_chunk", (double)h->task_pair_chunk}, {"threads", 0.0}};
     for (const auto& t : tab) if (!std::strcmp(name, t.n)) { *value = t.v; return 0; }
     FAIL(h, std::string("unknown option: ") + name);
 }
@@ -4761,6 +4825,7 @@
     HIPCK(h, hipMemcpyAsync(h->pinfo, info.data(), sizeof(float4) * h->Np, hipMemcpyHostToDevice, h->stream));
     HIPCK(h, hipStreamSynchronize(h->stream));
     h->tbl_of_frame[0] = 0;
+    h->hint_floor_serial = h->sort_serial;
     h->tail_used = true;
     h->keys_frame = -1;
     std::fill(h->fiso.begin(), h->fiso.end(), 0);
@@ -4859,6 +4924,7 @@
     CHECK_FRAME(h, f);
     if (f == h->keys_frame) h->keys_frame = -1;
     h->tail_used = true;
+    h->hint_floor_serial = h->sort_serial;
     h->gs_host_valid = false;
     if (h->gs_cap > 0) HIPCK(h, hipMemsetAsync(h->gs_flag + f, 0, sizeof(int), h->stream));
     if (F) h->fiso[f] = 0;
@@ -4879,6 +4945,7 @@
     CHECK_FRAME(h, f);
     if (f == h->keys_frame) h->keys_frame = -1;
     h->tail_used = true;
+    h->hint_floor_serial = h->sort_serial;
     h->gs_host_valid = false;
     if (h->gs_cap > 0) HIPCK(h, hipMemsetAsync(h->gs_flag + f, 0, sizeof(int), h->stream));
     const int mask = (x ? 1 : 0) | (v ? 2 : 0) | (C ? 4 : 0) | (F ? 8 : 0) | (used ? 16 : 0);
@@ -5309,14 +5376,19 @@
     out->n_slow_path = slow; out->bytes_state = (long long)h->bytes;
     return check_async(h);
 }
-int fe_get_work_stats(FeEngine* h, int f, long long out[FE_WORK_STATS]) { return fe_get_work_stats_n(h, f, out, FE_WORK_STATS); }
+int fe_get_work_stats(FeEngine* h, int f, long long out[24]) { return fe_get_work_stats_n(h, f, out, 24); }
 int fe_get_work_stats_n(FeEngine* h, int f, long long* out_, int n_out) {
     FE_ENTRY(h);
     CHECK_FRAME(h, f);
     if (!out_ || n_out < 0) FAIL(h, "fe_get_work_stats_n: bad output buffer");
     long long out[FE_WORK_STATS];
     struct Copy { long long* src; long long* dst; int n; ~Copy() { for (int i = 0; i < n && i < FE_WORK_STATS; i++) dst[i] = src[i]; } } copy_out{out, out_, n_out};
-    for (int i = 0; i < 24; i++) out[i] = 0;
+    for (int i = 0; i < FE_WORK_STATS; i++) out[i] = 0;
+    out[24] = out[27] = -1;
+    if ((size_t)f < h->gl_fwd.size()) {
+        const FeEngine::GridLaunchRec &a = h->gl_fwd[f], &b = h->gl_bwd[f];
+        out[23] = a.wgs; out[24] = a.hint; out[25] = a.kind; out[26] = b.wgs; out[27] = b.hint; out[28] = b.kind;
+    }
     const int t = h->tbl_of_frame[f];
     if (t < 0 || t >= (int)h->tables.size() || !h->tables[t].meta) return 0;
     int meta[16];
diff --git a/fluidlab_amd/csrc/fe_grid_launch.h b/fluidlab_amd/csrc/fe_grid_launch.h
--- /dev/null
+++ b/fluidlab_amd/csrc/fe_grid_launch.h
@@ -0,0 +1,34 @@
+#ifndef FE_GRID_LAUNCH_H
+#define FE_GRID_LAUNCH_H
+
+enum { FE_GL_NONE = 0, FE_GL_LAGGED = 1, FE_GL_EXACT = 2, FE_GL_FORCED = 3 };
+
+#define FE_GL_FIXED_WGS 1024
+#define FE_GL_FLOOR_WGS 512
+#define FE_GL_ONE_CAP_WGS 6144
+#define FE_GL_MARGIN_PCT 125
+#define FE_GL_QUANTUM 128
+
+inline int fe_grid_launch_fixed(int blocks, int cap) {
+    int g = (blocks + 3) / 4;
+    if (g < 1) g = 1;
+    const int c = cap > 0 ? cap : FE_GL_FIXED_WGS;
+    return g < c ? g : c;
+}
+
+inline int fe_grid_launch_wgs(long long hint, int margin_pct, bool exact, int blocks, int cap, int one_cap = FE_GL_ONE_CAP_WGS) {
+    const int fixed = fe_grid_launch_fixed(blocks, cap);
+    if (hint < 0) return fixed;
+    if (margin_pct < 100) margin_pct = 100;
+    const long long n = exact ? hint : (hint * margin_pct + 99) / 100;
+    long long g = (n + 3) / 4;
+    if (g > one_cap) return fixed;
+    if (g < FE_GL_FLOOR_WGS) g = FE_GL_FLOOR_WGS;
+    g = (g + FE_GL_QUANTUM - 1) / FE_GL_QUANTUM * FE_GL_QUANTUM;
+    const long long all = blocks > 4 ? (blocks + 3) / 4 : 1;
+    if (g > all) g = all;
+    if (cap > 0 && g > cap) g = cap;
+    return (int)g;
+}
+
+#endif
diff --git a/include/fluidengine.h b/include/fluidengine.h
--- a/include/fluidengine.h
+++ b/include/fluidengine.h
@@ -172,9 +172,9 @@
     long long bytes_state;
 } FeStats;
 int fe_get_stats(FeEngine* h, int f, FeStats* out);
-#define FE_WORK_STATS 24
+#define FE_WORK_STATS 30
 int fe_get_work_stats_n(FeEngine* h, int f, long long* out, int n);
-int fe_get_work_stats(FeEngine* h, int f, long long out[FE_WORK_STATS]);
+int fe_get_work_stats(FeEngine* h, int f, long long out[24]);
 int    fe_timer_start(FeEngine* h);
 double fe_timer_stop_ms(FeEngine* h);
 int fe_profile_enable(FeEngine* h, int on);
```

After: 11740 substep_pairs/s, median of 6. +2.5%, better.
